# unilight/jatts

Hardware: AMD Instinct MI355X
Metric: audio samples/sec (22.05 kHz) + RTF, FastSpeech2+HiFi-GAN (higher is better)
Workload: dtype f32 (emulated: 3 exact bf16 terms per operand, 7 MFMA products, f32 accumulate; attention / norms / duration predictor exact f32); 1 GPU; FastSpeech2(JSUT conformer 4+4, adim 384)+HiFi-GAN v1 22k, 64 utts x 128 phonemes x 6 frames per GPU; hop=256, parallelism=dp1 (utterance sharding, int16 PCM all-gather)

## Files before the change

include/jatts_hip.h:

```cpp
#ifndef JATTS_HIP_H_
#define JATTS_HIP_H_

#include <stdint.h>

#ifdef __cplusplus
extern "C" {
#endif

#define JATTS_ABI_VERSION 4

#define JATTS_F32 0
#define JATTS_F16 1
#define JATTS_F32S 2
#define JATTS_F32E 3
#define JATTS_F32E6 4

#define JATTS_ACT_NONE 0
#define JATTS_ACT_RELU 1
#define JATTS_ACT_TANH 2
#define JATTS_ACT_SWISH 3
#define JATTS_ACT_MISH 4
#define JATTS_ACT_SNAKEBETA 5

#define JATTS_PAD_ZERO 0
#define JATTS_PAD_REFLECT 1

#define JATTS_PRE_NONE 0
#define JATTS_PRE_LRELU 1

#define JATTS_OK 0
#define JATTS_ERR_ARG (-1)
#define JATTS_ERR_HIP (-2)
#define JATTS_ERR_UNSUPPORTED (-3)

int jatts_abi_version(void);
const char* jatts_last_error(void);
int jatts_device_info(char* buf, int buflen);

typedef struct jatts_ragged {
  const int32_t* cu_rows;
  int32_t n_seq;
  int32_t max_len;
  int32_t len_mul;
  int32_t total_rows;
  const int32_t* host_lens;
} jatts_ragged;

typedef struct jatts_conv_desc {
  jatts_ragged rg;
  int32_t dtype;
  int32_t n_in;
  const void* x[3];
  int32_t ldx;
  float in_scale;
  int32_t pre_act;
  float pre_slope;
  const void* w;
  int32_t c_in;
  int32_t n_out;
  int32_t k_w;
  int32_t dil;
  int32_t pad;
  const float* bias;
  int32_t act;
  float alpha;
  const float* resid;
  int32_t ldr;
  void* y;
  int32_t ldy;
  int32_t y_is_f32;
  int32_t y_transposed;
  const int32_t* y_seq_col0;
  int32_t pad_mode;
  int32_t variant;
  const float* w_inv;
  const float* act_a;
  const float* act_b;
  int32_t n_split;
  int32_t ldy2;
  void* y2;
  const int32_t* y2_seq_col0;
  int32_t w_layout;
} jatts_conv_desc;

int jatts_conv1d(const jatts_conv_desc* d, void* stream);

int64_t jatts_conv_weight_index(int32_t n, int32_t tap, int32_t c, int32_t n_pad, int32_t c_in);

typedef struct jatts_resunit_desc {
  jatts_ragged rg;
  int32_t dtype;
  int32_t channels;
  int32_t k_w;
  int32_t dil;
  float slope;
  const void* x;
  void* y;
  const void* w1;
  const float* b1;
  const void* w2;
  const float* b2;
  const void* add0;
  const void* add1;
  float out_scale;
  const float* ws1;
  const float* ws2;
  int32_t w_layout;
} jatts_resunit_desc;

int jatts_hifigan_resunit(const jatts_resunit_desc* d, void* stream);

int64_t jatts_unit_weight_index_k32(int32_t n, int32_t tap, int32_t c, int32_t channels);

typedef struct jatts_resblock_desc {
  jatts_ragged rg;
  int32_t dtype;
  int32_t channels;
  int32_t k_w;
  int32_t n_units;
  int32_t dil[3];
  float slope;
  const void* x;
  void* y;
  const void* w1[3];
  const float* b1[3];
  const void* w2[3];
  const float* b2[3];
  const void* add0;
  const void* add1;
  float out_scale;
  const float* ws1[3];
  const float* ws2[3];
} jatts_resblock_desc;

int jatts_hifigan_resblock(const jatts_resblock_desc* d, void* stream);

int jatts_masked_loss(const jatts_ragged* rg, const float* a, int32_t lda, const float* b, int32_t ldb, int32_t dim,
                      const int32_t* valid_len, int32_t kind, float log_offset, double scale, float* out, double* workspace,
                      void* stream);
int jatts_conv1d_wgrad(const jatts_ragged* rg, const float* x, int32_t ldx, const float* dy, int32_t ldy, int32_t c_in,
                       int32_t n_out, int32_t k_w, int32_t dil, int32_t pad, float* dw, float* db, float* workspace, void* stream);
int jatts_pack_conv_weight(const float* w, int32_t n_out, int32_t c_in, int32_t k_w, int32_t c_mult, int32_t mode, int32_t dtype,
                           void* out, void* stream);
int jatts_pack_conv_weight_split(const float* w, int32_t n_out, int32_t c_in, int32_t k_w, int32_t c_mult, int32_t mode, void* out, float* inv,
                                 void* stream);
int jatts_col_sum(const float* x, int32_t ld, int64_t rows, int32_t dim, float* out, void* stream);

int jatts_layernorm_bwd(const float* x, int32_t ldx, const float* dy, int32_t lddy, const float* gamma, int64_t rows, int32_t dim,
                        float eps, float* dx, int32_t lddx, float* dgamma, float* dbeta, void* stream);
int jatts_act_fwd(int32_t mode, const float* x, float* y, int64_t n, void* stream);
int jatts_act_bwd(int32_t mode, const float* x, const float* dy, float* dx, int64_t n, void* stream);
int jatts_glu_fwd(const float* x, float* y, int64_t rows, int32_t dim, void* stream);
int jatts_glu_bwd(const float* x, const float* dy, float* dx, int64_t rows, int32_t dim, void* stream);
int jatts_dwconv(const jatts_ragged* rg, const float* x, const float* w, const float* bias, float* y, int32_t dim, int32_t k_w,
                 int32_t pad, int32_t flip, void* stream);
int jatts_dwconv_wgrad(const jatts_ragged* rg, const float* x, const float* dy, float* dw, int32_t dim, int32_t k_w, int32_t pad,
                       void* stream);
int jatts_col_stats(const float* x, const float* y2, int32_t ld, int64_t rows, int32_t dim, const float* shift, const float* mul,
                    int32_t mode, float* out0, float* out1, void* stream);
int jatts_bn_bwd_apply(const float* x, const float* dy, int64_t rows, int32_t dim, const float* mean, const float* rstd,
                       const float* gamma, const float* s_dy, const float* s_dyx, float* dx, void* stream);
int jatts_index_add_rows(const float* src, int32_t ld, const int64_t* idx, int64_t rows, int32_t dim, float scale, int64_t skip,
                         int64_t n_dst, float* dst, void* stream);
int jatts_lr_segment_sum(const jatts_ragged* rg, const int64_t* cum, const int32_t* cu_out, const float* dy, int32_t dim, float* dhs,
                         void* stream);
int jatts_shift_softmax_fwd(const float* ac, const float* bd, int32_t n_batch, int32_t n_heads, int32_t t_len, const int32_t* lens,
                            float scale, int32_t shift_mode, float* p, void* stream);
int jatts_shift_softmax_bwd(const float* p, const float* dp, int32_t n_batch, int32_t n_heads, int32_t t_len, float scale,
                            int32_t shift_mode, float* ds, float* dbd, void* stream);
int jatts_gate_bwd(const float* x, const float* dy, float* dx, int64_t rows, int32_t dim, void* stream);
int jatts_weight_norm_fwd(const float* v, const float* g, int32_t n_out, int32_t row_len, float* w, float* inv_norm, void* stream);
int jatts_weight_norm_bwd(const float* v, const float* g, const float* inv_norm, const float* dw, int32_t n_out, int32_t row_len,
                          float* dv, float* dg, void* stream);
int jatts_split_add(const float* o, const float* h, const float* skip, int64_t rows, int32_t dim, float* h_out, float* skip_out, void* stream);
int jatts_concat2(const float* a, const float* b, int64_t rows, int32_t dim, float* out, void* stream);
int jatts_outer_rows(const float* v, const float* w, const float* bias, int64_t rows, int32_t dim, int32_t accumulate, float* out,
                     void* stream);
int jatts_col_wsum(const float* x, int32_t ld, const float* v, int64_t rows, int32_t dim, float* out, void* stream);
int jatts_row_dot(const float* x, int32_t ld, const float* w, const float* bias, int64_t rows, int32_t dim, float* y, void* stream);
int jatts_masked_loss_bwd(const jatts_ragged* rg, const float* a, int32_t lda, const float* b, int32_t ldb, int32_t dim,
                          const int32_t* valid_len, int32_t kind, float log_offset, float scale, const float* upstream, float* da,
                          int32_t ldda, void* stream);
int jatts_groupnorm_fwd(const jatts_ragged* rg, const float* x, int32_t dim, int32_t groups, const float* gamma, const float* beta,
                        float eps, float* y, float* mean, float* rstd, void* stream);
int jatts_groupnorm_bwd(const jatts_ragged* rg, const float* x, const float* dy, int32_t dim, int32_t groups, const float* gamma,
                        const float* mean, const float* rstd, float* dx, float* dgamma, float* dbeta, void* stream);
int jatts_snakebeta_fwd(const float* x, float* y, int64_t rows, int32_t dim, const float* alpha, const float* beta, void* stream);
int jatts_snakebeta_bwd(const float* x, const float* dy, int64_t rows, int32_t dim, const float* alpha, const float* beta, float* dx,
                        float* dalpha, float* dbeta, void* stream);
int jatts_ctc_forward_sum(const float* log_p, int32_t n_batch, int32_t t_max, int32_t ld, const int32_t* ilens, const int32_t* olens,
                          int32_t max_ilen, float log_blank, float* workspace, float* nll, float* grad, float grad_scale, void* stream);
int jatts_seq_sum(const jatts_ragged* rg, const float* x, int32_t dim, float* out, void* stream);
int jatts_dropout(const float* x, float* y, int64_t n, float p, uint64_t seed, const uint64_t* seed_dev, void* stream);
int jatts_qkv_split(const float* qkv, const float* u, const float* v, int32_t n_batch, int32_t t_len, int32_t n_heads, int32_t d_k, float* qu,
                    float* qv, float* k, float* vv, void* stream);
int jatts_qkv_split_bwd(const float* dqu, const float* dqv, const float* dk, const float* dvv, int32_t n_batch, int32_t t_len, int32_t n_heads,
                        int32_t d_k, float* dqkv, float* du, float* dv, void* stream);
int jatts_act_dropout(int32_t mode, const float* x, const float* dy, float* out, int64_t n, float p, uint64_t seed, const uint64_t* seed_dev,
                      void* stream);
int jatts_dropout_add(const float* x, const float* resid, float* y, int64_t n, float p, float alpha, uint64_t seed, const uint64_t* seed_dev,
                      void* stream);
int jatts_gather_grads(const float* const* src, const int64_t* numel, const int64_t* dst_off, int32_t n, float* flat, int32_t accumulate,
                       void* stream);
int jatts_sumsq(const float* x, int64_t n, double* out, void* stream);
int jatts_adam_step(float* p, const float* g, float* m, float* v, int64_t n, double lr, double beta1, double beta2, double eps,
                    double weight_decay, int64_t step, const double* grad_sumsq, float max_norm, const float* hyper_dev, void* stream);

int jatts_debug_trace(void* buf, int64_t n_workgroups);

int jatts_mfma_probe(int32_t dtype, int32_t feed, const void* operands, int64_t operand_bytes, int32_t iters, int32_t workgroups,
                     uint64_t* clocks, float* sink, void* stream);
double jatts_mfma_probe_flops(int32_t dtype, int32_t iters, int32_t workgroups);

int jatts_bgemm(const float* a, int64_t sa_outer, int64_t sa_inner, int32_t lda, int32_t trans_a, const float* b, int64_t sb_outer,
                int64_t sb_inner, int32_t ldb, int32_t trans_b, float* c, int64_t sc_outer, int64_t sc_inner, int32_t ldc, int32_t n_outer,
                int32_t n_inner, int32_t m, int32_t n, int32_t k, float alpha, int32_t accumulate, void* stream);

int jatts_set_workspace(void* buf, int64_t bytes);

int jatts_hifigan_output(const jatts_ragged* rg, int32_t dtype, const void* const* x, int32_t n_in,
                         float in_scale, float slope, int32_t c_in, int32_t k_w, const float* w,
                         float bias, float* y, void* stream);

typedef struct jatts_relattn_desc {
  jatts_ragged rg;
  int32_t dtype;
  int32_t n_heads;
  int32_t d_k;
  const void* q;  int32_t ldq;
  const void* k;  int32_t ldk;
  const void* vt; int32_t ldvt;
  const void* g;  int32_t ldg;
  const float* ku;
  float scale;
  void* out; int32_t ldo;
  int32_t rel_mode;
  int32_t rel_center;
  const int32_t* vt_col0;
  const int32_t* kv_len;
} jatts_relattn_desc;

int jatts_relpos_attention(const jatts_relattn_desc* d, void* stream);

int jatts_rowdot(int32_t dtype, const void* x, int32_t ldx, int64_t rows, int32_t n_heads,
                 int32_t d_k, const float* vec, float* out, void* stream);

int jatts_embed_scale(const int64_t* ids, int64_t rows, const float* table, int32_t dim,
                      float scale, float* out, int64_t vocab, int64_t* n_bad, void* stream);

int jatts_layernorm(const void* x, int32_t in_dtype, int32_t ldx, void* y, int32_t out_dtype,
                    int32_t ldy, int64_t rows, int32_t dim, const float* gamma,
                    const float* beta, float eps, void* stream);

int jatts_affine_cast(const float* x, int32_t ldx, void* y, int32_t out_dtype, int32_t ldy,
                      int64_t rows, int32_t dim, const float* scale, const float* shift,
                      void* stream);
int jatts_affine_slice(const float* x, int32_t ldx, void* y, int32_t out_dtype, int32_t ldy,
                      int64_t rows, int32_t dim, const float* scale, const float* shift,
                      void* stream);

int jatts_glu_dwconv_bn_swish(const jatts_ragged* rg, int32_t dtype, const void* x, void* y,
                              int32_t channels, int32_t k_w, const float* w_dw,
                              const float* bn_scale, const float* bn_shift, void* stream);

int jatts_predictor_head(int32_t dtype, const void* x, int32_t ldx, int64_t rows, int32_t dim,
                         const float* w, float b, float* v_out, int64_t* dur_out, float offset,
                         void* stream);

int jatts_variance_embed_add(const jatts_ragged* rg, float* hs, int32_t dim, const float* p,
                             const float* wp, const float* bp, int32_t kp, const float* e,
                             const float* we, const float* be, int32_t ke, void* stream);

int jatts_gated_tanh_sigmoid(const jatts_ragged* rg, int32_t dtype, const void* x, const float* gseq,
                             void* y, int32_t channels, void* stream);

int jatts_groupnorm_mish(const jatts_ragged* rg, const void* x, int32_t in_dtype, void* y, int32_t out_dtype,
                         int32_t channels, int32_t groups, const float* gamma, const float* beta, float eps,
                         const float* addvec, float* workspace, void* stream);

int jatts_snakebeta(int32_t dtype, const void* x, void* y, int64_t rows, int32_t channels, const float* alpha,
                    const float* inv_beta, void* stream);

int jatts_l2_normalize(const float* x, int32_t ldx, void* y, int32_t out_dtype, int32_t ldy, int64_t rows,
                       int32_t dim, float eps, void* stream);

int jatts_gaussian_sample(const float* stats, const float* noise, float* z, int64_t rows, int32_t channels,
                          float noise_scale, void* stream);

int jatts_flip_channels(const float* x, float* y, int64_t rows, int32_t channels, void* stream);

int jatts_add_seq_vector(const jatts_ragged* rg, float* hs, int32_t dim, const float* vec,
                         void* stream);

int jatts_frame_signal(const jatts_ragged* rg_frames, const int32_t* cu_samples, const float* x, const float* window,
                       int32_t n_fft, int32_t hop, float* out, int32_t ldo, void* stream);
int jatts_power_spectrum(const float* x, int32_t ldx, int32_t n_bins, int64_t rows, float* out, int32_t ldo, void* stream);
int jatts_fbank_post(const jatts_ragged* rg, const float* p, int32_t ldp, int32_t n_mels, float amin, float top_db,
                     float* out, int32_t ldo, void* stream);
int jatts_seq_mean_std(const jatts_ragged* rg, const float* x, int32_t ldx, int32_t dim, const float* logits, int32_t ldl,
                       float* mean, float* stdv, int32_t ldm, float eps, void* stream);
int jatts_seq_affine_act(const jatts_ragged* rg, const float* x, int32_t ldx, int32_t dim, const float* seq_vec, int32_t pre_act,
                         const float* scale, const float* shift, int32_t post_act, void* y, int32_t out_dtype, int32_t ldy,
                         void* stream);
int jatts_se_scale_add(const jatts_ragged* rg, const float* x, int32_t dim, const float* s, const float* resid, float* y, int32_t ldy,
                       void* stream);

int jatts_lr_durations(const jatts_ragged* rg, const int64_t* d, float alpha, int32_t zero_rule,
                       int64_t* d_eff, int64_t* cum, int64_t* olens, void* stream);
int jatts_lr_gather(const jatts_ragged* rg_in, const int64_t* cum, const int32_t* cu_out,
                    int32_t max_out_len, const float* x, int32_t dim, float* out,
                    int64_t* frame_index, void* stream);

int jatts_zero_pad_rows(const jatts_ragged* rg, void* x, int32_t dtype, int32_t ld, int32_t dim, const int32_t* valid_len,
                        void* stream);
int jatts_cfm_mix(const jatts_ragged* rg, const float* x1, const float* z, const float* t, float sigma_min, int32_t dim,
                  float* y, float* u, void* stream);
int jatts_sq_err_sum(const float* a, const float* b, int64_t n, float scale, float* out, double* workspace, void* stream);

int jatts_gaussian_upsample(const jatts_ragged* rg_in, const int64_t* d, const int32_t* cu_out,
                            int32_t max_out_len, const float* hs, int32_t dim, float delta,
                            float* out, void* stream);

int jatts_pcm16(const float* x, int64_t n, int16_t* y, void* stream);

int jatts_alignment_logp(const jatts_ragged* rg_feats, const int32_t* cu_text, int32_t max_text_len, const float* feats,
                         const float* text, int32_t adim, float* log_p, int32_t ld, void* stream);

int jatts_mas_viterbi(const jatts_ragged* rg_feats, const int32_t* cu_text, const float* log_p, int32_t ld,
                      int32_t max_text_len, int64_t* path, int64_t* dur, double* score, void* stream);

#ifdef __cplusplus
}
#endif
#endif
```

jatts_amd/_abi.py:

```python
import ctypes as C
import os

_HERE = os.path.dirname(os.path.abspath(__file__))
LIB_PATH = os.environ.get("JATTS_HIP_LIB") or os.path.join(_HERE, "lib", "libjatts_hip.so")

F32, F16, F32S, F32E, F32E6 = 0, 1, 2, 3, 4
ABI_VERSION = 4
ACT_NONE, ACT_RELU, ACT_TANH, ACT_SWISH, ACT_MISH, ACT_SNAKEBETA = 0, 1, 2, 3, 4, 5
PRE_NONE, PRE_LRELU = 0, 1
PAD_ZERO, PAD_REFLECT = 0, 1


class Ragged(C.Structure):
    _fields_ = [("cu_rows", C.c_void_p), ("n_seq", C.c_int32), ("max_len", C.c_int32),
                ("len_mul", C.c_int32), ("total_rows", C.c_int32), ("host_lens", C.c_void_p)]


class ConvDesc(C.Structure):
    _fields_ = [
        ("rg", Ragged), ("dtype", C.c_int32), ("n_in", C.c_int32), ("x", C.c_void_p * 3),
        ("ldx", C.c_int32), ("in_scale", C.c_float), ("pre_act", C.c_int32), ("pre_slope", C.c_float),
        ("w", C.c_void_p), ("c_in", C.c_int32), ("n_out", C.c_int32), ("k_w", C.c_int32),
        ("dil", C.c_int32), ("pad", C.c_int32), ("bias", C.c_void_p), ("act", C.c_int32),
        ("alpha", C.c_float), ("resid", C.c_void_p), ("ldr", C.c_int32), ("y", C.c_void_p),
        ("ldy", C.c_int32), ("y_is_f32", C.c_int32), ("y_transposed", C.c_int32), ("y_seq_col0", C.c_void_p),
        ("pad_mode", C.c_int32), ("variant", C.c_int32), ("w_inv", C.c_void_p), ("act_a", C.c_void_p), ("act_b", C.c_void_p),
        ("n_split", C.c_int32), ("ldy2", C.c_int32), ("y2", C.c_void_p), ("y2_seq_col0", C.c_void_p), ("w_layout", C.c_int32),
    ]


class ResUnitDesc(C.Structure):
    _fields_ = [
        ("rg", Ragged), ("dtype", C.c_int32), ("channels", C.c_int32), ("k_w", C.c_int32),
        ("dil", C.c_int32), ("slope", C.c_float), ("x", C.c_void_p), ("y", C.c_void_p),
        ("w1", C.c_void_p), ("b1", C.c_void_p), ("w2", C.c_void_p), ("b2", C.c_void_p),
        ("add0", C.c_void_p), ("add1", C.c_void_p), ("out_scale", C.c_float),
        ("ws1", C.c_void_p), ("ws2", C.c_void_p), ("w_layout", C.c_int32),
    ]


class ResBlockDesc(C.Structure):
    _fields_ = [
        ("rg", Ragged), ("dtype", C.c_int32), ("channels", C.c_int32), ("k_w", C.c_int32), ("n_units", C.c_int32),
        ("dil", C.c_int32 * 3), ("slope", C.c_float), ("x", C.c_void_p), ("y", C.c_void_p),
        ("w1", C.c_void_p * 3), ("b1", C.c_void_p * 3), ("w2", C.c_void_p * 3), ("b2", C.c_void_p * 3),
        ("add0", C.c_void_p), ("add1", C.c_void_p), ("out_scale", C.c_float),
        ("ws1", C.c_void_p * 3), ("ws2", C.c_void_p * 3),
    ]


class RelAttnDesc(C.Structure):
    _fields_ = [
        ("rg", Ragged), ("dtype", C.c_int32), ("n_heads", C.c_int32), ("d_k", C.c_int32),
        ("q", C.c_void_p), ("ldq", C.c_int32), ("k", C.c_void_p), ("ldk", C.c_int32),
        ("vt", C.c_void_p), ("ldvt", C.c_int32), ("g", C.c_void_p), ("ldg", C.c_int32),
        ("ku", C.c_void_p), ("scale", C.c_float), ("out", C.c_void_p), ("ldo", C.c_int32),
        ("rel_mode", C.c_int32), ("rel_center", C.c_int32), ("vt_col0", C.c_void_p), ("kv_len", C.c_void_p),
    ]


PROTOTYPES = {
    "jatts_abi_version": (C.c_int, []),
    "jatts_last_error": (C.c_char_p, []),
    "jatts_device_info": (C.c_int, [C.c_char_p, C.c_int]),
    "jatts_conv1d": (C.c_int, [C.POINTER(ConvDesc), C.c_void_p]),
    "jatts_conv_weight_index": (C.c_int64, [C.c_int32] * 5),
    "jatts_hifigan_resunit": (C.c_int, [C.POINTER(ResUnitDesc), C.c_void_p]),
    "jatts_unit_weight_index_k32": (C.c_int64, [C.c_int32] * 4),
    "jatts_hifigan_resblock": (C.c_int, [C.POINTER(ResBlockDesc), C.c_void_p]),
    "jatts_debug_trace": (C.c_int, [C.c_void_p, C.c_int64]),
    "jatts_mfma_probe": (C.c_int, [C.c_int32, C.c_int32, C.c_void_p, C.c_int64, C.c_int32, C.c_int32, C.c_void_p, C.c_void_p, C.c_void_p]),
    "jatts_mfma_probe_flops": (C.c_double, [C.c_int32, C.c_int32, C.c_int32]),
    "jatts_set_workspace": (C.c_int, [C.c_void_p, C.c_int64]),
    "jatts_pack_conv_weight_split": (C.c_int, [C.c_void_p, C.c_int32, C.c_int32, C.c_int32, C.c_int32, C.c_int32, C.c_void_p, C.c_void_p, C.c_void_p]),
    "jatts_bgemm": (C.c_int, [C.c_void_p, C.c_int64, C.c_int64, C.c_int32, C.c_int32, C.c_void_p, C.c_int64, C.c_int64, C.c_int32, C.c_int32,
                              C.c_void_p, C.c_int64, C.c_int64, C.c_int32, C.c_int32, C.c_int32, C.c_int32, C.c_int32, C.c_int32, C.c_float,
                              C.c_int32, C.c_void_p]),
    "jatts_pcm16": (C.c_int, [C.c_void_p, C.c_int64, C.c_void_p, C.c_void_p]),
    "jatts_alignment_logp": (C.c_int, [C.POINTER(Ragged), C.c_void_p, C.c_int32, C.c_void_p, C.c_void_p, C.c_int32,
                                       C.c_void_p, C.c_int32, C.c_void_p]),
    "jatts_mas_viterbi": (C.c_int, [C.POINTER(Ragged), C.c_void_p, C.c_void_p, C.c_int32, C.c_int32, C.c_void_p,
                                    C.c_void_p, C.c_void_p, C.c_void_p]),
    "jatts_hifigan_output": (C.c_int, [C.POINTER(Ragged), C.c_int32, C.POINTER(C.c_void_p), C.c_int32,
                                       C.c_float, C.c_float, C.c_int32, C.c_int32, C.c_void_p, C.c_float,
                                       C.c_void_p, C.c_void_p]),
    "jatts_relpos_attention": (C.c_int, [C.POINTER(RelAttnDesc), C.c_void_p]),
    "jatts_rowdot": (C.c_int, [C.c_int32, C.c_void_p, C.c_int32, C.c_int64, C.c_int32, C.c_int32,
                               C.c_void_p, C.c_void_p, C.c_void_p]),
    "jatts_embed_scale": (C.c_int, [C.c_void_p, C.c_int64, C.c_void_p, C.c_int32, C.c_float, C.c_void_p,
                                    C.c_int64, C.c_void_p, C.c_void_p]),
    "jatts_layernorm": (C.c_int, [C.c_void_p, C.c_int32, C.c_int32, C.c_void_p, C.c_int32, C.c_int32,
                                  C.c_int64, C.c_int32, C.c_void_p, C.c_void_p, C.c_float, C.c_void_p]),
    "jatts_affine_cast": (C.c_int, [C.c_void_p, C.c_int32, C.c_void_p, C.c_int32, C.c_int32, C.c_int64,
                                    C.c_int32, C.c_void_p, C.c_void_p, C.c_void_p]),
    "jatts_affine_slice": (C.c_int, [C.c_void_p, C.c_int32, C.c_void_p, C.c_int32, C.c_int32, C.c_int64,
                                     C.c_int32, C.c_void_p, C.c_void_p, C.c_void_p]),
    "jatts_glu_dwconv_bn_swish": (C.c_int, [C.POINTER(Ragged), C.c_int32, C.c_void_p, C.c_void_p, C.c_int32,
                                            C.c_int32, C.c_void_p, C.c_void_p, C.c_void_p, C.c_void_p]),
    "jatts_predictor_head": (C.c_int, [C.c_int32, C.c_void_p, C.c_int32, C.c_int64, C.c_int32, C.c_void_p,
                                       C.c_float, C.c_void_p, C.c_void_p, C.c_float, C.c_void_p]),
    "jatts_variance_embed_add": (C.c_int, [C.POINTER(Ragged), C.c_void_p, C.c_int32, C.c_void_p, C.c_void_p,
                                           C.c_void_p, C.c_int32, C.c_void_p, C.c_void_p, C.c_void_p,
                                           C.c_int32, C.c_void_p]),
    "jatts_gated_tanh_sigmoid": (C.c_int, [C.POINTER(Ragged), C.c_int32, C.c_void_p, C.c_void_p, C.c_void_p,
                                           C.c_int32, C.c_void_p]),
    "jatts_groupnorm_mish": (C.c_int, [C.POINTER(Ragged), C.c_void_p, C.c_int32, C.c_void_p, C.c_int32, C.c_int32,
                                       C.c_int32, C.c_void_p, C.c_void_p, C.c_float, C.c_void_p, C.c_void_p, C.c_void_p]),
    "jatts_snakebeta": (C.c_int, [C.c_int32, C.c_void_p, C.c_void_p, C.c_int64, C.c_int32, C.c_void_p, C.c_void_p,
                                  C.c_void_p]),
    "jatts_l2_normalize": (C.c_int, [C.c_void_p, C.c_int32, C.c_void_p, C.c_int32, C.c_int32, C.c_int64, C.c_int32,
                                     C.c_float, C.c_void_p]),
    "jatts_gaussian_sample": (C.c_int, [C.c_void_p, C.c_void_p, C.c_void_p, C.c_int64, C.c_int32, C.c_float,
                                        C.c_void_p]),
    "jatts_flip_channels": (C.c_int, [C.c_void_p, C.c_void_p, C.c_int64, C.c_int32, C.c_void_p]),
    "jatts_add_seq_vector": (C.c_int, [C.POINTER(Ragged), C.c_void_p, C.c_int32, C.c_void_p, C.c_void_p]),
    "jatts_lr_durations": (C.c_int, [C.POINTER(Ragged), C.c_void_p, C.c_float, C.c_int32, C.c_void_p,
                                     C.c_void_p, C.c_void_p, C.c_void_p]),
    "jatts_lr_gather": (C.c_int, [C.POINTER(Ragged), C.c_void_p, C.c_void_p, C.c_int32, C.c_void_p,
                                  C.c_int32, C.c_void_p, C.c_void_p, C.c_void_p]),
    "jatts_frame_signal": (C.c_int, [C.POINTER(Ragged), C.c_void_p, C.c_void_p, C.c_void_p, C.c_int32, C.c_int32, C.c_void_p,
                                     C.c_int32, C.c_void_p]),
    "jatts_power_spectrum": (C.c_int, [C.c_void_p, C.c_int32, C.c_int32, C.c_int64, C.c_void_p, C.c_int32, C.c_void_p]),
    "jatts_fbank_post": (C.c_int, [C.POINTER(Ragged), C.c_void_p, C.c_int32, C.c_int32, C.c_float, C.c_float, C.c_void_p,
                                   C.c_int32, C.c_void_p]),
    "jatts_seq_mean_std": (C.c_int, [C.POINTER(Ragged), C.c_void_p, C.c_int32, C.c_int32, C.c_void_p, C.c_int32, C.c_void_p,
                                     C.c_void_p, C.c_int32, C.c_float, C.c_void_p]),
    "jatts_seq_affine_act": (C.c_int, [C.POINTER(Ragged), C.c_void_p, C.c_int32, C.c_int32, C.c_void_p, C.c_int32, C.c_void_p,
                                       C.c_void_p, C.c_int32, C.c_void_p, C.c_int32, C.c_int32, C.c_void_p]),
    "jatts_se_scale_add": (C.c_int, [C.POINTER(Ragged), C.c_void_p, C.c_int32, C.c_void_p, C.c_void_p, C.c_void_p, C.c_int32,
                                     C.c_void_p]),
    "jatts_masked_loss": (C.c_int, [C.POINTER(Ragged), C.c_void_p, C.c_int32, C.c_void_p, C.c_int32, C.c_int32, C.c_void_p,
                                    C.c_int32, C.c_float, C.c_double, C.c_void_p, C.c_void_p, C.c_void_p]),
    "jatts_conv1d_wgrad": (C.c_int, [C.POINTER(Ragged), C.c_void_p, C.c_int32, C.c_void_p, C.c_int32, C.c_int32, C.c_int32,
                                     C.c_int32, C.c_int32, C.c_int32, C.c_void_p, C.c_void_p, C.c_void_p, C.c_void_p]),
    "jatts_pack_conv_weight": (C.c_int, [C.c_void_p, C.c_int32, C.c_int32, C.c_int32, C.c_int32, C.c_int32, C.c_int32, C.c_void_p, C.c_void_p]),
    "jatts_col_sum": (C.c_int, [C.c_void_p, C.c_int32, C.c_int64, C.c_int32, C.c_void_p, C.c_void_p]),
    "jatts_layernorm_bwd": (C.c_int, [C.c_void_p, C.c_int32, C.c_void_p, C.c_int32, C.c_void_p, C.c_int64, C.c_int32, C.c_float, C.c_void_p, C.c_int32, C.c_void_p, C.c_void_p, C.c_void_p]),
    "jatts_act_fwd": (C.c_int, [C.c_int32, C.c_void_p, C.c_void_p, C.c_int64, C.c_void_p]),
    "jatts_act_bwd": (C.c_int, [C.c_int32, C.c_void_p, C.c_void_p, C.c_void_p, C.c_int64, C.c_void_p]),
    "jatts_glu_fwd": (C.c_int, [C.c_void_p, C.c_void_p, C.c_int64, C.c_int32, C.c_void_p]),
    "jatts_glu_bwd": (C.c_int, [C.c_void_p, C.c_void_p, C.c_void_p, C.c_int64, C.c_int32, C.c_void_p]),
    "jatts_dwconv": (C.c_int, [C.POINTER(Ragged), C.c_void_p, C.c_void_p, C.c_void_p, C.c_void_p, C.c_int32, C.c_int32, C.c_int32, C.c_int32, C.c_void_p]),
    "jatts_dwconv_wgrad": (C.c_int, [C.POINTER(Ragged), C.c_void_p, C.c_void_p, C.c_void_p, C.c_int32, C.c_int32, C.c_int32, C.c_void_p]),
    "jatts_col_stats": (C.c_int, [C.c_void_p, C.c_void_p, C.c_int32, C.c_int64, C.c_int32, C.c_void_p, C.c_void_p, C.c_int32, C.c_void_p, C.c_void_p, C.c_void_p]),
    "jatts_bn_bwd_apply": (C.c_int, [C.c_void_p, C.c_void_p, C.c_int64, C.c_int32, C.c_void_p, C.c_void_p, C.c_void_p, C.c_void_p, C.c_void_p, C.c_void_p, C.c_void_p]),
    "jatts_index_add_rows": (C.c_int, [C.c_void_p, C.c_int32, C.c_void_p, C.c_int64, C.c_int32, C.c_float, C.c_int64, C.c_int64, C.c_void_p, C.c_void_p]),
    "jatts_lr_segment_sum": (C.c_int, [C.POINTER(Ragged), C.c_void_p, C.c_void_p, C.c_void_p, C.c_int32, C.c_void_p, C.c_void_p]),
    "jatts_shift_softmax_fwd": (C.c_int, [C.c_void_p, C.c_void_p, C.c_int32, C.c_int32, C.c_int32, C.c_void_p, C.c_float, C.c_int32, C.c_void_p, C.c_void_p]),
    "jatts_shift_softmax_bwd": (C.c_int, [C.c_void_p, C.c_void_p, C.c_int32, C.c_int32, C.c_int32, C.c_float, C.c_int32, C.c_void_p, C.c_void_p, C.c_void_p]),
    "jatts_gate_bwd": (C.c_int, [C.c_void_p, C.c_void_p, C.c_void_p, C.c_int64, C.c_int32, C.c_void_p]),
    "jatts_weight_norm_fwd": (C.c_int, [C.c_void_p, C.c_void_p, C.c_int32, C.c_int32, C.c_void_p, C.c_void_p, C.c_void_p]),
    "jatts_weight_norm_bwd": (C.c_int, [C.c_void_p, C.c_void_p, C.c_void_p, C.c_void_p, C.c_int32, C.c_int32, C.c_void_p, C.c_void_p, C.c_void_p]),
    "jatts_split_add": (C.c_int, [C.c_void_p, C.c_void_p, C.c_void_p, C.c_int64, C.c_int32, C.c_void_p, C.c_void_p, C.c_void_p]),
    "jatts_concat2": (C.c_int, [C.c_void_p, C.c_void_p, C.c_int64, C.c_int32, C.c_void_p, C.c_void_p]),
    "jatts_outer_rows": (C.c_int, [C.c_void_p, C.c_void_p, C.c_void_p, C.c_int64, C.c_int32, C.c_int32, C.c_void_p, C.c_void_p]),
    "jatts_col_wsum": (C.c_int, [C.c_void_p, C.c_int32, C.c_void_p, C.c_int64, C.c_int32, C.c_void_p, C.c_void_p]),
    "jatts_row_dot": (C.c_int, [C.c_void_p, C.c_int32, C.c_void_p, C.c_void_p, C.c_int64, C.c_int32, C.c_void_p, C.c_void_p]),
    "jatts_masked_loss_bwd": (C.c_int, [C.POINTER(Ragged), C.c_void_p, C.c_int32, C.c_void_p, C.c_int32, C.c_int32, C.c_void_p, C.c_int32, C.c_float, C.c_float, C.c_void_p, C.c_void_p, C.c_int32, C.c_void_p]),
    "jatts_groupnorm_fwd": (C.c_int, [C.POINTER(Ragged), C.c_void_p, C.c_int32, C.c_int32, C.c_void_p, C.c_void_p, C.c_float, C.c_void_p, C.c_void_p, C.c_void_p, C.c_void_p]),
    "jatts_groupnorm_bwd": (C.c_int, [C.POINTER(Ragged), C.c_void_p, C.c_void_p, C.c_int32, C.c_int32, C.c_void_p, C.c_void_p, C.c_void_p, C.c_void_p, C.c_void_p, C.c_void_p, C.c_void_p]),
    "jatts_snakebeta_fwd": (C.c_int, [C.c_void_p, C.c_void_p, C.c_int64, C.c_int32, C.c_void_p, C.c_void_p, C.c_void_p]),
    "jatts_snakebeta_bwd": (C.c_int, [C.c_void_p, C.c_void_p, C.c_int64, C.c_int32, C.c_void_p, C.c_void_p, C.c_void_p, C.c_void_p, C.c_void_p, C.c_void_p]),
    "jatts_ctc_forward_sum": (C.c_int, [C.c_void_p, C.c_int32, C.c_int32, C.c_int32, C.c_void_p, C.c_void_p, C.c_int32, C.c_float, C.c_void_p, C.c_void_p, C.c_void_p, C.c_float, C.c_void_p]),
    "jatts_seq_sum": (C.c_int, [C.POINTER(Ragged), C.c_void_p, C.c_int32, C.c_void_p, C.c_void_p]),
    "jatts_dropout": (C.c_int, [C.c_void_p, C.c_void_p, C.c_int64, C.c_float, C.c_uint64, C.c_void_p, C.c_void_p]),
    "jatts_qkv_split": (C.c_int, [C.c_void_p, C.c_void_p, C.c_void_p, C.c_int32, C.c_int32, C.c_int32, C.c_int32, C.c_void_p, C.c_void_p, C.c_void_p, C.c_void_p, C.c_void_p]),
    "jatts_qkv_split_bwd": (C.c_int, [C.c_void_p, C.c_void_p, C.c_void_p, C.c_void_p, C.c_int32, C.c_int32, C.c_int32, C.c_int32, C.c_void_p, C.c_void_p, C.c_void_p, C.c_void_p]),
    "jatts_act_dropout": (C.c_int, [C.c_int32, C.c_void_p, C.c_void_p, C.c_void_p, C.c_int64, C.c_float, C.c_uint64, C.c_void_p, C.c_void_p]),
    "jatts_dropout_add": (C.c_int, [C.c_void_p, C.c_void_p, C.c_void_p, C.c_int64, C.c_float, C.c_float, C.c_uint64, C.c_void_p, C.c_void_p]),
    "jatts_sumsq": (C.c_int, [C.c_void_p, C.c_int64, C.c_void_p, C.c_void_p]),
    "jatts_gather_grads": (C.c_int, [C.c_void_p, C.c_void_p, C.c_void_p, C.c_int32, C.c_void_p, C.c_int32, C.c_void_p]),
    "jatts_adam_step": (C.c_int, [C.c_void_p, C.c_void_p, C.c_void_p, C.c_void_p, C.c_int64, C.c_double, C.c_double, C.c_double, C.c_double, C.c_double, C.c_int64, C.c_void_p, C.c_float, C.c_void_p, C.c_void_p]),
    "jatts_zero_pad_rows": (C.c_int, [C.POINTER(Ragged), C.c_void_p, C.c_int32, C.c_int32, C.c_int32, C.c_void_p, C.c_void_p]),
    "jatts_cfm_mix": (C.c_int, [C.POINTER(Ragged), C.c_void_p, C.c_void_p, C.c_void_p, C.c_float, C.c_int32, C.c_void_p,
                                C.c_void_p, C.c_void_p]),
    "jatts_sq_err_sum": (C.c_int, [C.c_void_p, C.c_void_p, C.c_int64, C.c_float, C.c_void_p, C.c_void_p, C.c_void_p]),
    "jatts_gaussian_upsample": (C.c_int, [C.POINTER(Ragged), C.c_void_p, C.c_void_p, C.c_int32, C.c_void_p,
                                          C.c_int32, C.c_float, C.c_void_p, C.c_void_p]),
}

_lib = None


class JattsHipError(RuntimeError):
    pass


def load():
    global _lib
    if _lib is not None:
        return _lib
    if not os.path.exists(LIB_PATH):
        raise JattsHipError(
            f"{LIB_PATH} not found: build it with `python -c 'import __graft_entry__ as g; g.build()'` "
            "or `make -C jatts_amd/csrc`.  jatts_amd has no CPU fallback."
        )
    lib = C.CDLL(LIB_PATH)
    for name, (res, args) in PROTOTYPES.items():
        fn = getattr(lib, name)
        fn.restype, fn.argtypes = res, args
    if lib.jatts_abi_version() != ABI_VERSION:
        raise JattsHipError(f"libjatts_hip.so ABI version {lib.jatts_abi_version()} != {ABI_VERSION} (include/jatts_hip.h): rebuild with __graft_entry__.build()")
    _lib = lib
    return lib


def check(rc, what=""):
    if rc != 0:
        msg = load().jatts_last_error().decode(errors="replace")
        raise JattsHipError(f"{what} failed (rc={rc}): {msg}")
```

jatts_amd/csrc/conv_api.hip:

```cpp
#include <stdlib.h>

#include "common.h"

unsigned long long* jatts_g_trace = nullptr;
unsigned jatts_g_trace_cap = 0;

int jatts_conv1d_f16(const jatts_conv_desc& d, hipStream_t s);
int jatts_conv1d_f32(const jatts_conv_desc& d, hipStream_t s);
int jatts_conv1d_split(const jatts_conv_desc& d, hipStream_t s);
int jatts_conv1d_emul(const jatts_conv_desc& d, hipStream_t s);
int jatts_resunit_f16_narrow(const jatts_resunit_desc& d, hipStream_t s);
int jatts_resunit_f16_wide(const jatts_resunit_desc& d, hipStream_t s);
int jatts_resunit_f32(const jatts_resunit_desc& d, hipStream_t s);
int jatts_resunit_split(const jatts_resunit_desc& d, hipStream_t s);
int jatts_resunit_emul(const jatts_resunit_desc& d, hipStream_t s);
int jatts_resblock_f16(const jatts_resblock_desc& d, hipStream_t s);
int jatts_resblock_f32(const jatts_resblock_desc& d, hipStream_t s);
int jatts_resblock_split(const jatts_resblock_desc& d, hipStream_t s);
int jatts_resblock_emul(const jatts_resblock_desc& d, hipStream_t s);

extern "C" int jatts_debug_trace(void* buf, int64_t n_workgroups) {
  jatts_g_trace = (unsigned long long*)buf;
  jatts_g_trace_cap = buf ? (unsigned)n_workgroups : 0u;
  return JATTS_OK;
}

extern "C" int64_t jatts_conv_weight_index(int32_t n, int32_t tap, int32_t c, int32_t n_pad, int32_t c_in) {
  const int64_t KC16 = c_in / 16, NFR = n_pad / 32;
  const int64_t kc = c / 16, nf = n / 32;
  const int64_t lane = 32 * ((c % 16) / 8) + (n % 32);
  return ((((int64_t)tap * KC16 + kc) * NFR + nf) * 64 + lane) * 8 + (c % 8);
}

extern "C" int64_t jatts_unit_weight_index_k32(int32_t n, int32_t tap, int32_t c, int32_t channels) {
  const int64_t KC32 = channels / 32, NFR16 = channels / 16;
  const int64_t kc = c / 32, nf = n / 16;
  const int64_t lane = 16 * ((c % 32) / 8) + (n % 16);
  return ((((int64_t)tap * KC32 + kc) * NFR16 + nf) * 64 + lane) * 8 + (c % 8);
}

extern "C" int jatts_conv1d(const jatts_conv_desc* d, void* stream) {
  if (!d || !d->x[0] || !d->w || !d->y || !d->rg.cu_rows) return jatts_set_error_msg(JATTS_ERR_ARG, "conv1d: null pointer");
  if (d->c_in <= 0 || d->c_in % 64) return jatts_set_error_msg(JATTS_ERR_ARG, "conv1d: c_in must be a positive multiple of 64");
  if (d->ldx % 8) return jatts_set_error_msg(JATTS_ERR_ARG, "conv1d: ldx must be a multiple of 8");
  if (d->n_in < 1 || d->n_in > 3 || d->k_w < 1 || d->dil < 1 || d->n_out < 1 || d->rg.n_seq < 1 || d->rg.len_mul < 1)
    return jatts_set_error_msg(JATTS_ERR_ARG, "conv1d: bad geometry");
  if (d->act == JATTS_ACT_SNAKEBETA && (!d->act_a || !d->act_b || (d->n_out & 3) || ((uintptr_t)d->act_a & 15) || ((uintptr_t)d->act_b & 15)))
    return jatts_set_error_msg(JATTS_ERR_ARG, "conv1d: JATTS_ACT_SNAKEBETA needs 16-byte aligned act_a / act_b and n_out % 4 == 0");
  if (d->n_split != 0 && (d->n_split < 0 || d->n_split % 256 || d->n_split >= d->n_out || !d->y2 || d->y_transposed || d->resid || d->ldy2 <= 0))
    return jatts_set_error_msg(JATTS_ERR_ARG, "conv1d: n_split must be a multiple of 256 below n_out, with y2 / ldy2 set, y row-major and no residual");
  if (d->w_layout != 0 && d->dtype != JATTS_F32E && d->dtype != JATTS_F32E6) return jatts_set_error_msg(JATTS_ERR_ARG, "conv1d: w_layout = 1 goes with JATTS_F32E / JATTS_F32E6 only");
  if (d->rg.max_len <= 0) return JATTS_OK;
  hipStream_t s = (hipStream_t)stream;
  if (d->dtype == JATTS_F16) return jatts_conv1d_f16(*d, s);
  if (d->dtype == JATTS_F32) return jatts_conv1d_f32(*d, s);
  if (d->dtype == JATTS_F32S) {
    if (!d->w_inv) return jatts_set_error_msg(JATTS_ERR_ARG, "conv1d: JATTS_F32S needs w_inv");
    if (!d->y_is_f32) return jatts_set_error_msg(JATTS_ERR_ARG, "conv1d: JATTS_F32S writes f32 (y_is_f32 = 1)");
    return jatts_conv1d_split(*d, s);
  }
  if (d->dtype == JATTS_F32E || d->dtype == JATTS_F32E6) {
    if (!d->y_is_f32) return jatts_set_error_msg(JATTS_ERR_ARG, "conv1d: JATTS_F32E / JATTS_F32E6 write f32 (y_is_f32 = 1)");
    if (d->w_layout != 0 && d->w_layout != 1) return jatts_set_error_msg(JATTS_ERR_ARG, "conv1d: w_layout must be 0 or 1");
    return jatts_conv1d_emul(*d, s);
  }
  return jatts_set_error_msg(JATTS_ERR_ARG, "conv1d: unknown dtype");
}

extern "C" int jatts_hifigan_resunit(const jatts_resunit_desc* d, void* stream) {
  if (!d || !d->x || !d->y || !d->w1 || !d->w2 || !d->b1 || !d->b2 || !d->rg.cu_rows)
    return jatts_set_error_msg(JATTS_ERR_ARG, "resunit: null pointer");
  if (d->x == d->y) return jatts_set_error_msg(JATTS_ERR_ARG, "resunit: y must not alias x");
  if (d->k_w < 1 || !(d->k_w & 1) || d->dil < 1) return jatts_set_error_msg(JATTS_ERR_ARG, "resunit: odd k_w and dil>=1 required");
  if (!(d->slope >= 0.f && d->slope <= 1.f)) return jatts_set_error_msg(JATTS_ERR_ARG, "resunit: LeakyReLU slope must be in [0, 1]");
  if (d->rg.max_len <= 0) return JATTS_OK;
  hipStream_t s = (hipStream_t)stream;
  if (d->dtype == JATTS_F16) return d->channels <= 64 ? jatts_resunit_f16_narrow(*d, s) : jatts_resunit_f16_wide(*d, s);
  if (d->dtype == JATTS_F32) return jatts_resunit_f32(*d, s);
  if (d->dtype == JATTS_F32S) {
    if (!d->ws1 || !d->ws2) return jatts_set_error_msg(JATTS_ERR_ARG, "resunit: JATTS_F32S needs ws1 / ws2");
    return jatts_resunit_split(*d, s);
  }
  if (d->dtype == JATTS_F32E || d->dtype == JATTS_F32E6) {
    if (d->w_layout != 0 && d->w_layout != 1) return jatts_set_error_msg(JATTS_ERR_ARG, "resunit: w_layout must be 0 or 1");
    return jatts_resunit_emul(*d, s);
  }
  if (d->w_layout != 0) return jatts_set_error_msg(JATTS_ERR_ARG, "resunit: w_layout = 1 goes with JATTS_F32E / JATTS_F32E6 only");
  return jatts_set_error_msg(JATTS_ERR_UNSUPPORTED, "resunit: unsupported channels/dtype (use jatts_conv1d)");
}

extern "C" int jatts_hifigan_resblock(const jatts_resblock_desc* d, void* stream) {
  if (!d || !d->x || !d->y || !d->rg.cu_rows) return jatts_set_error_msg(JATTS_ERR_ARG, "resblock: null pointer");
  if (d->n_units < 1 || d->n_units > 3) return jatts_set_error_msg(JATTS_ERR_ARG, "resblock: 1..3 units");
  for (int u = 0; u < d->n_units; ++u) {
    if (!d->w1[u] || !d->w2[u] || !d->b1[u] || !d->b2[u]) return jatts_set_error_msg(JATTS_ERR_ARG, "resblock: null weights");
    if (d->dil[u] < 1) return jatts_set_error_msg(JATTS_ERR_ARG, "resblock: dil >= 1 required");
  }
  if (d->x == d->y) return jatts_set_error_msg(JATTS_ERR_ARG, "resblock: y must not alias x");
  if (d->k_w < 1 || !(d->k_w & 1)) return jatts_set_error_msg(JATTS_ERR_ARG, "resblock: odd k_w required");
  if (!(d->slope >= 0.f && d->slope <= 1.f)) return jatts_set_error_msg(JATTS_ERR_ARG, "resblock: LeakyReLU slope must be in [0, 1]");
  if (d->dtype == JATTS_F32S) {
    for (int u = 0; u < d->n_units; ++u)
      if (!d->ws1[u] || !d->ws2[u]) return jatts_set_error_msg(JATTS_ERR_ARG, "resblock: JATTS_F32S needs ws1 / ws2");
    if (d->rg.max_len <= 0) return JATTS_OK;
    return jatts_resblock_split(*d, (hipStream_t)stream);
  }
  if (d->dtype == JATTS_F32E || d->dtype == JATTS_F32E6) {
    if (d->rg.max_len <= 0) return JATTS_OK;
    return jatts_resblock_emul(*d, (hipStream_t)stream);
  }
  if (d->dtype != JATTS_F16 && d->dtype != JATTS_F32) return jatts_set_error_msg(JATTS_ERR_ARG, "resblock: unknown dtype");
  if (d->rg.max_len <= 0) return JATTS_OK;
  return d->dtype == JATTS_F16 ? jatts_resblock_f16(*d, (hipStream_t)stream) : jatts_resblock_f32(*d, (hipStream_t)stream);
}
```

jatts_amd/csrc/resunit_emul.hip:

```cpp
#include "resunit_emul16_impl.h"

template <typename T>
static int resunit_emul(const jatts_resunit_desc& d, hipStream_t s) {
  const int halo = (d.k_w - 1) * d.dil;
  const int64_t cols = (int64_t)d.rg.max_len * d.rg.len_mul;
  auto wgs = [&](int window) { const int64_t tt = window - (d.k_w - 1); return tt > 0 ? ((cols + tt - 1) / tt) * d.rg.n_seq : (int64_t)1 << 40; };
  switch (d.channels) {
    case 32: return launch_resunit_emul<T, 32, 256, 1, 2, 2, 2, false, true>(d, s);
    case 64:
      if (d.k_w >= 11) return launch_resunit_emul<T, 64, 256, 1, 2, 2, 1, false, true>(d, s);
      return launch_resunit_emul<T, 64, 128, 2, 2, 2, 2, false, true>(d, s);
    case 128:
      if (wgs(128) <= 448 && (64 + halo) * 784 + 1024 <= 80 * 1024) return launch_resunit_emul<T, 128, 64, 2, 1, 2, 2>(d, s);
      return launch_resunit_emul<T, 128, 128, 2, 2, 2, 1>(d, s);
    case 256:
      if (wgs(64) <= 160) return launch_resunit_emul<T, 256, 32, 4, 1, 2, 1>(d, s);
      if ((64 + halo) * 1552 + 2048 <= 160 * 1024) return launch_resunit_emul<T, 256, 64, 4, 2, 2, 1>(d, s);
      return launch_resunit_emul<T, 256, 64, 4, 2, 2, 1, true>(d, s);
  }
  return jatts_set_error_msg(JATTS_ERR_UNSUPPORTED, "resunit: unsupported channels for JATTS_F32E (32 / 64 / 128 / 256)");
}

template <typename T>
static int resunit_emul16(const jatts_resunit_desc& d, hipStream_t s) {
  const int halo = (d.k_w - 1) * d.dil;
  switch (d.channels) {
    case 32: return launch_resunit_emul16<T, 32, 256, 1, 4, 2, false, true>(d, s);
    case 64:
      if (d.k_w >= 11) return launch_resunit_emul16<T, 64, 256, 1, 4, 1, false, true>(d, s);
      return launch_resunit_emul16<T, 64, 128, 2, 2, 2, false, true>(d, s);
    case 128: return launch_resunit_emul16<T, 128, 128, 2, 2, 1>(d, s);
    case 256:
      if ((64 + halo) * 1552 + 2048 <= 160 * 1024) return launch_resunit_emul16<T, 256, 64, 4, 1, 1>(d, s);
      return launch_resunit_emul16<T, 256, 64, 4, 1, 1, true>(d, s);
  }
  return jatts_set_error_msg(JATTS_ERR_UNSUPPORTED, "resunit: unsupported channels for JATTS_F32E (32 / 64 / 128 / 256)");
}

int jatts_resunit_emul(const jatts_resunit_desc& d, hipStream_t s) {
  if (d.w_layout == 1) return d.dtype == JATTS_F32E6 ? resunit_emul16<bf3f>(d, s) : resunit_emul16<bf3>(d, s);
  return d.dtype == JATTS_F32E6 ? resunit_emul<bf3f>(d, s) : resunit_emul<bf3>(d, s);
}
```

jatts_amd/csrc/resunit_emul16_impl.h:

```cpp
#pragma once
#include <type_traits>

#include "resunit_emul_impl.h"

#ifndef JATTS_U16_ROWS
#define JATTS_U16_ROWS 1
#endif
#ifndef JATTS_U16_DIAG
#define JATTS_U16_DIAG 0
#endif

namespace {

struct acc2x4 { f32x4 big, small; };
template <typename T> struct Acc16 { typedef f32x4 type; };
template <> struct Acc16<bf3p<7>> { typedef acc2x4 type; };
__device__ __forceinline__ void acc16_set(f32x4& a, int i, float v) { a[i] = v; }
__device__ __forceinline__ void acc16_set(acc2x4& a, int i, float v) { a.small[i] = v; a.big[i] = 0.f; }
__device__ __forceinline__ void acc16_finish(f32x4&) {}
__device__ __forceinline__ void acc16_finish(acc2x4& a) { a.small = a.big + a.small; }
__device__ __forceinline__ f32x4& acc16_val(f32x4& a) { return a; }
__device__ __forceinline__ f32x4& acc16_val(acc2x4& a) { return a.small; }

template <int P> __device__ __forceinline__ void mma16p(const bf3px8<7>& a, const bf3px8<7>& b, acc2x4& c) {
  if constexpr (P == 0) c.small = __builtin_amdgcn_mfma_f32_16x16x32_bf16(a.b1, b.b2, c.small, 0, 0, 0);
  if constexpr (P == 1) c.small = __builtin_amdgcn_mfma_f32_16x16x32_bf16(a.b2, b.b0, c.small, 0, 0, 0);
  if constexpr (P == 2) c.small = __builtin_amdgcn_mfma_f32_16x16x32_bf16(a.b0, b.b2, c.small, 0, 0, 0);
  if constexpr (P == 3) c.small = __builtin_amdgcn_mfma_f32_16x16x32_bf16(a.b1, b.b1, c.small, 0, 0, 0);
  if constexpr (P == 4) c.small = __builtin_amdgcn_mfma_f32_16x16x32_bf16(a.b1, b.b0, c.small, 0, 0, 0);
  if constexpr (P == 5) c.small = __builtin_amdgcn_mfma_f32_16x16x32_bf16(a.b0, b.b1, c.small, 0, 0, 0);
  if constexpr (P == 6) c.big = __builtin_amdgcn_mfma_f32_16x16x32_bf16(a.b0, b.b0, c.big, 0, 0, 0);
}
template <int P> __device__ __forceinline__ void mma16p(const bf3px8<6>& a, const bf3px8<6>& b, f32x4& c) {
  if constexpr (P == 0) c = __builtin_amdgcn_mfma_f32_16x16x32_bf16(a.b2, b.b0, c, 0, 0, 0);
  if constexpr (P == 1) c = __builtin_amdgcn_mfma_f32_16x16x32_bf16(a.b0, b.b2, c, 0, 0, 0);
  if constexpr (P == 2) c = __builtin_amdgcn_mfma_f32_16x16x32_bf16(a.b1, b.b1, c, 0, 0, 0);
  if constexpr (P == 3) c = __builtin_amdgcn_mfma_f32_16x16x32_bf16(a.b1, b.b0, c, 0, 0, 0);
  if constexpr (P == 4) c = __builtin_amdgcn_mfma_f32_16x16x32_bf16(a.b0, b.b1, c, 0, 0, 0);
  if constexpr (P == 5) c = __builtin_amdgcn_mfma_f32_16x16x32_bf16(a.b0, b.b0, c, 0, 0, 0);
}
template <typename T> struct NProd;
template <int NP> struct NProd<bf3p<NP>> { static constexpr int value = NP; };

template <typename T, int NF>
struct WStream16 {
  typedef typename Elem<T>::vec8 V8;
  V8 ra[NF];
  const T* wl;
  int kc_stride;
  int tap_stride;
  __device__ __forceinline__ void bind(const T* w, int KC32, int NFR16, int nf0, int lane) {
    wl = w + (size_t)nf0 * 512 + (size_t)lane * 8;
    kc_stride = NFR16 * 512;
    tap_stride = KC32 * kc_stride;
  }
  __device__ __forceinline__ void fetch(int tap, int kc) {
    const T* p = wl + (size_t)tap * tap_stride + (size_t)kc * kc_stride;
#pragma unroll
    for (int f = 0; f < NF; ++f) ra[f] = Vec8IO<T>::ldg(p + f * 512);
  }
};

template <typename T, int NF, int NT>
__device__ __forceinline__ void pair16(typename Acc16<T>::type (&acc)[NF][NT], const typename Elem<T>::vec8& a, typename Elem<T>::vec8 (&rb)[NT], int f_, int t0_) {
  constexpr int NP = NProd<T>::value;
  auto& c0 = acc[f_][t0_];
  auto& c1 = acc[f_][t0_ + 1];
  mma16p<0>(a, rb[t0_], c0); mma16p<0>(a, rb[t0_ + 1], c1);
  mma16p<1>(a, rb[t0_], c0); mma16p<1>(a, rb[t0_ + 1], c1);
  mma16p<2>(a, rb[t0_], c0); mma16p<2>(a, rb[t0_ + 1], c1);
  mma16p<3>(a, rb[t0_], c0); mma16p<3>(a, rb[t0_ + 1], c1);
  mma16p<4>(a, rb[t0_], c0); mma16p<4>(a, rb[t0_ + 1], c1);
  mma16p<5>(a, rb[t0_], c0); mma16p<5>(a, rb[t0_ + 1], c1);
  if constexpr (NP == 7) { mma16p<6>(a, rb[t0_], c0); mma16p<6>(a, rb[t0_ + 1], c1); }
}

template <typename T, int NF, int NT>
__device__ __forceinline__ void row16(typename Acc16<T>::type (&acc)[NF][NT], const typename Elem<T>::vec8& a, typename Elem<T>::vec8 (&rb)[NT], int f_) {
  constexpr int NP = NProd<T>::value;
#pragma unroll
  for (int t = 0; t < NT; ++t) mma16p<0>(a, rb[t], acc[f_][t]);
#pragma unroll
  for (int t = 0; t < NT; ++t) mma16p<1>(a, rb[t], acc[f_][t]);
#pragma unroll
  for (int t = 0; t < NT; ++t) mma16p<2>(a, rb[t], acc[f_][t]);
#pragma unroll
  for (int t = 0; t < NT; ++t) mma16p<3>(a, rb[t], acc[f_][t]);
#pragma unroll
  for (int t = 0; t < NT; ++t) mma16p<4>(a, rb[t], acc[f_][t]);
#pragma unroll
  for (int t = 0; t < NT; ++t) mma16p<5>(a, rb[t], acc[f_][t]);
  if constexpr (NP == 7) {
#pragma unroll
    for (int t = 0; t < NT; ++t) mma16p<6>(a, rb[t], acc[f_][t]);
  }
}

template <typename T, int NF, int NT>
__device__ __forceinline__ void step16(typename Acc16<T>::type (&acc)[NF][NT], typename Elem<T>::vec8 (&ra)[NF], typename Elem<T>::vec8 (&rb)[NT], const T* pa,
                                       const char* pb, int pitch) {
  static_assert(NT % 2 == 0, "column fragments come in pairs");
  constexpr bool ROWS16 = JATTS_U16_ROWS != 0;
#pragma unroll
  for (int f = 0; f < NF; ++f) {
    if (f < NF - 1 && ROWS16) {
      row16<T, NF, NT>(acc, ra[f], rb, f);
      __builtin_amdgcn_sched_barrier(0);
    } else {
#pragma unroll
      for (int tp = 0; tp < NT; tp += 2) {
        pair16<T, NF, NT>(acc, ra[f], rb, f, tp);
        if (f == NF - 1 && !(JATTS_U16_DIAG & 1)) {
          rb[tp] = Vec8IO<T>::lds(pb + (size_t)(tp * 16) * pitch);
          rb[tp + 1] = Vec8IO<T>::lds(pb + (size_t)((tp + 1) * 16) * pitch);
        }
        __builtin_amdgcn_sched_barrier(0);
      }
    }
    if (!(JATTS_U16_DIAG & 2)) ra[f] = Vec8IO<T>::ldg(pa + f * 512);
    __builtin_amdgcn_sched_barrier(0);
  }
}

template <typename T, int NF, int NT, int KCS>
__device__ __forceinline__ void conv16(typename Acc16<T>::type (&acc)[NF][NT], WStream16<T, NF>& ws, int kc0, int k_w, int dil, const char* act, int pitch,
                                       int col0, int lane, const T* tail) {
  typedef typename Elem<T>::vec8 V8;
  const int steps = k_w * KCS;
  const char* bbase = act + (size_t)(col0 + (lane & 15)) * pitch + (size_t)(lane >> 4) * 48;
  const T* abase = ws.wl + (size_t)kc0 * ws.kc_stride;
  V8 rb[NT];
#pragma unroll
  for (int t = 0; t < NT; ++t) rb[t] = Vec8IO<T>::lds(bbase + (size_t)(t * 16) * pitch);
  __builtin_amdgcn_sched_barrier(0);
  if (!tail) tail = abase + (size_t)(k_w - 1) * ws.tap_stride + (size_t)(KCS - 1) * ws.kc_stride;
  int tap = 0, kk = 0;
  for (int s = 0; s < steps; ++s) {
    int nkk = kk + 1;
    const bool wrap = nkk == KCS;
    nkk = wrap ? 0 : nkk;
    const int ntap = tap + (wrap ? 1 : 0);
    const bool last = s + 1 >= steps;
    const T* pa = last ? tail : abase + (size_t)ntap * ws.tap_stride + (size_t)nkk * ws.kc_stride;
    const char* pb = bbase + (size_t)((last ? tap : ntap) * dil) * pitch + (size_t)((last ? kk : nkk) * 4) * 48;
    step16<T, NF, NT>(acc, ws.ra, rb, pa, pb, pitch);
    tap = ntap;
    kk = nkk;
  }
}

template <typename T, int C, int WGCOLS, int WN, int WT, int OCC, bool KSPLIT = false, bool RREG = false>
__global__ __launch_bounds__(WN* WT * 64, OCC) void resunit_emul16_kernel(jatts_resunit_desc d, unsigned long long* trace, unsigned trace_cap,
                                                                         unsigned bias_off) {
  typedef typename Elem<T>::vec8 V8;
  extern __shared__ __attribute__((aligned(16))) char smem[];
  constexpr int NF = C / (WN * 16), NT = WGCOLS / (WT * 16);
  constexpr int KC32 = C / 32, NFR16 = C / 16;
  constexpr int pitch = C * 6 + 16;
  constexpr int pitch_x = KSPLIT ? (C / 2) * 6 + 16 : pitch;
  constexpr int NTHR = WN * WT * 64;
  static_assert(NF * WN * 16 == C && NT * WT * 16 == WGCOLS && C % 32 == 0, "tile shape");
  static_assert(sizeof(T) == 6, "bf3 is three packed bf16");
  static_assert(!(KSPLIT && RREG), "the residual registers go with the one-piece x tile");
  static_assert(!KSPLIT || KC32 % 2 == 0, "channel halves are whole K-steps");
  constexpr int MAXI = RREG ? (WGCOLS * (C / 8) + NTHR - 1) / NTHR : 1;
  f32x8 xk[MAXI];
  const unsigned wg_lin = blockIdx.x + blockIdx.y * gridDim.x;
  const bool tracing = trace != nullptr && wg_lin < trace_cap && threadIdx.x == 0;
#define JATTS_STAMP(i) do { if (tracing) trace[(size_t)wg_lin * 16 + (i)] = __builtin_amdgcn_s_memtime(); } while (0)
  if (tracing) {
    unsigned hwid, xcc;
    asm volatile("s_getreg_b32 %0, hwreg(HW_REG_HW_ID)" : "=s"(hwid));
    asm volatile("s_getreg_b32 %0, hwreg(HW_REG_XCC_ID)" : "=s"(xcc));
    trace[(size_t)wg_lin * 16] = ((unsigned long long)xcc << 32) | hwid;
    trace[(size_t)wg_lin * 16 + 8] = __builtin_amdgcn_s_memrealtime();
  }
  JATTS_STAMP(1);
  const int K = d.k_w, dil = d.dil;
  const int p2 = (K - 1) / 2, p1 = p2 * dil;
  const int tt_out = WGCOLS - 2 * p2;

  int b = blockIdx.y, bx = blockIdx.x;
  if (ragged_is_1d(d.rg) && !ragged_locate(d.rg, tt_out, blockIdx.x, b, bx)) return;
  const int row_b = d.rg.cu_rows[b];
  const int L = (d.rg.cu_rows[b + 1] - row_b) * d.rg.len_mul;
  const int t0 = bx * tt_out;
  if (t0 >= L) return;
  const int64_t seq_row0 = (int64_t)row_b * d.rg.len_mul;
  const int lane = threadIdx.x & 63, wave = threadIdx.x >> 6;
  const int wn = wave / WT, wt = wave % WT;
  const int g4 = lane >> 4;
  const int col0 = wt * NT * 16;
  const int nf0 = wn * NF;

  const int rx = WGCOLS + 2 * p1;
  char* xs = smem;
  char* hs = smem;
  float* bs = reinterpret_cast<float*>(smem + bias_off);
  for (int u = threadIdx.x; u < 2 * C; u += NTHR) bs[u] = u < C ? d.b1[u] : d.b2[u - C];

  WStream16<T, NF> ws;
  ws.bind((const T*)d.w1, KC32, NFR16, nf0, lane);
  ws.fetch(0, 0);

  typename Acc16<T>::type acc[NF][NT];
  auto bias_acc = [&](const float* bv) {
#pragma unroll
    for (int f = 0; f < NF; ++f) {
      const f32x4 bb = *reinterpret_cast<const f32x4*>(bv + (nf0 + f) * 16 + 4 * g4);
#pragma unroll
      for (int t = 0; t < NT; ++t)
#pragma unroll
        for (int e = 0; e < 4; ++e) acc16_set(acc[f][t], e, bb[e]);
    }
  };
  auto finish_acc = [&]() {
#pragma unroll
    for (int f = 0; f < NF; ++f)
#pragma unroll
      for (int t = 0; t < NT; ++t) acc16_finish(acc[f][t]);
  };
  auto to_planes = [&](f32x8 v) {
    lrelu8(v, d.slope);
    V8 o;
    bf3_split8(v, o);
    return o;
  };
  const float* x = (const float*)d.x;
  const int pos0 = t0 - p2 - p1;
  if constexpr (!KSPLIT) {
    constexpr int UPR = C / 8;
    constexpr int UB = 8;
    const int total = rx * UPR;
    if constexpr (RREG) {
      const int r_in = p1 + p2, n_in = tt_out * UPR;
#pragma unroll
      for (int j = 0; j < MAXI; ++j) {
        const int v = threadIdx.x + j * NTHR;
        const int ro = v / UPR, cu = v - ro * UPR;
        const int pos = t0 + ro;
        if (v < n_in && pos < L) xk[j] = Vec8IO<float>::ldg(x + (seq_row0 + pos) * (int64_t)C + cu * 8);
        else xk[j] = f32x8{0, 0, 0, 0, 0, 0, 0, 0};
      }
      const int n_halo = (rx - tt_out) * UPR;
      for (int base = threadIdx.x; base < n_halo; base += NTHR * UB) {
        f32x8 v[UB];
#pragma unroll
        for (int j = 0; j < UB; ++j) {
          const int u = base + j * NTHR;
          int r = u / UPR;
          const int cu = u - r * UPR;
          if (r >= r_in) r += tt_out;
          const int pos = pos0 + r;
          if (u < n_halo && pos >= 0 && pos < L) v[j] = Vec8IO<float>::ldg(x + (seq_row0 + pos) * (int64_t)C + cu * 8);
          else v[j] = f32x8{0, 0, 0, 0, 0, 0, 0, 0};
        }
#pragma unroll
        for (int j = 0; j < UB; ++j) {
          const int u = base + j * NTHR;
          if (u >= n_halo) continue;
          int r = u / UPR;
          const int cu = u - r * UPR;
          if (r >= r_in) r += tt_out;
          Vec8IO<T>::sts(xs + (size_t)r * pitch + (size_t)cu * 48, to_planes(v[j]));
        }
      }
#pragma unroll
      for (int j = 0; j < MAXI; ++j) {
        const int v = threadIdx.x + j * NTHR;
        if (v >= n_in) continue;
        const int ro = v / UPR, cu = v - ro * UPR;
        Vec8IO<T>::sts(xs + (size_t)(r_in + ro) * pitch + (size_t)cu * 48, to_planes(xk[j]));
      }
    } else {
      constexpr int UBX = ((WGCOLS + 64) * UPR + NTHR - 1) / NTHR;
      for (int base = threadIdx.x; base < total; base += NTHR * UBX) {
        f32x8 v[UBX];
#pragma unroll
        for (int j = 0; j < UBX; ++j) {
          const int u = base + j * NTHR;
          const int r = u / UPR, cu = u - r * UPR;
          const int pos = pos0 + r;
          if (u < total && pos >= 0 && pos < L) v[j] = Vec8IO<float>::ldg(x + (seq_row0 + pos) * (int64_t)C + cu * 8);
          else v[j] = f32x8{0, 0, 0, 0, 0, 0, 0, 0};
        }
#pragma unroll
        for (int j = 0; j < UBX; ++j) {
          const int u = base + j * NTHR;
          if (u >= total) continue;
          const int r = u / UPR, cu = u - r * UPR;
          Vec8IO<T>::sts(xs + (size_t)r * pitch + (size_t)cu * 48, to_planes(v[j]));
        }
      }
    }
    __syncthreads();
    JATTS_STAMP(2);
    bias_acc(bs);
    conv16<T, NF, NT, KC32>(acc, ws, 0, K, dil, xs, pitch, col0, lane, (const T*)d.w2 + (size_t)nf0 * 512 + (size_t)lane * 8);
  } else {
    constexpr int UPR = C / 16;
    constexpr int MAXU = ((WGCOLS + 64) * UPR + NTHR - 1) / NTHR;
    const int total = rx * UPR;
    f32x8 xv[MAXU];
    auto load_half = [&](int half) {
#pragma unroll
      for (int j = 0; j < MAXU; ++j) {
        const int u = threadIdx.x + j * NTHR;
        const int r = u / UPR, cu = u - r * UPR;
        const int pos = pos0 + r;
        if (u < total && pos >= 0 && pos < L) xv[j] = Vec8IO<float>::ldg(x + (seq_row0 + pos) * (int64_t)C + half * (C / 2) + cu * 8);
        else xv[j] = f32x8{0, 0, 0, 0, 0, 0, 0, 0};
      }
    };
    auto store_half = [&]() {
#pragma unroll
      for (int j = 0; j < MAXU; ++j) {
        const int u = threadIdx.x + j * NTHR;
        if (u < total) Vec8IO<T>::sts(xs + (size_t)(u / UPR) * pitch_x + (size_t)(u % UPR) * 48, to_planes(xv[j]));
      }
    };
    load_half(0);
    store_half();
    load_half(1);
    __syncthreads();
    JATTS_STAMP(2);
    bias_acc(bs);
    conv16<T, NF, NT, KC32 / 2>(acc, ws, 0, K, dil, xs, pitch_x, col0, lane, ws.wl + (size_t)(KC32 / 2) * ws.kc_stride);
    lds_barrier();
    store_half();
    lds_barrier();
    conv16<T, NF, NT, KC32 / 2>(acc, ws, KC32 / 2, K, dil, xs, pitch_x, col0, lane, (const T*)d.w2 + (size_t)nf0 * 512 + (size_t)lane * 8);
  }
  finish_acc();
  JATTS_STAMP(3);

  lds_barrier();
  JATTS_STAMP(10);
  for (int u = threadIdx.x; u < (K - 1) * (C / 8); u += NTHR) {
    const int r = WGCOLS + u / (C / 8), cu = u % (C / 8);
    V8 z;
#pragma unroll
    for (int e = 0; e < 8; ++e) z.b0[e] = z.b1[e] = z.b2[e] = (bf16)0.f;
    Vec8IO<T>::sts(hs + (size_t)r * pitch + (size_t)cu * 48, z);
  }
#pragma unroll
  for (int t = 0; t < NT; ++t) {
    const int col = col0 + t * 16 + (lane & 15);
    const int pos = t0 - p2 + col;
    const float keep = (pos >= 0 && pos < L) ? 1.f : 0.f;
#pragma unroll
    for (int f = 0; f < NF; ++f) {
      const int n0 = (nf0 + f) * 16 + 4 * g4;
      float v[4];
#pragma unroll
      for (int e = 0; e < 4; ++e) {
        const float a = acc16_val(acc[f][t])[e] * keep;
        v[e] = fmaxf(a, a * d.slope);
      }
      bf16x4 q0, q1, q2;
      bf3_split4(v, q0, q1, q2);
      char* p = hs + (size_t)col * pitch + (size_t)(n0 >> 3) * 48 + (size_t)(n0 & 4) * 2;
      *reinterpret_cast<bf16x4*>(p) = q0;
      *reinterpret_cast<bf16x4*>(p + 16) = q1;
      *reinterpret_cast<bf16x4*>(p + 32) = q2;
    }
  }
  JATTS_STAMP(12);
  lds_barrier();
  JATTS_STAMP(4);

  bias_acc(bs + C);
  ws.bind((const T*)d.w2, KC32, NFR16, nf0, lane);
  conv16<T, NF, NT, KC32>(acc, ws, 0, K, 1, hs, pitch, col0, lane, nullptr);
  finish_acc();
  JATTS_STAMP(5);

  __syncthreads();
  char* ys = smem;
#pragma unroll
  for (int t = 0; t < NT; ++t) {
    const int col = col0 + t * 16 + (lane & 15);
    if (col >= tt_out || t0 + col >= L) continue;
#pragma unroll
    for (int f = 0; f < NF; ++f) {
      const int n0 = (nf0 + f) * 16 + 4 * g4;
      *reinterpret_cast<f32x4*>(ys + (size_t)col * pitch + (size_t)n0 * 4) = acc16_val(acc[f][t]);
    }
  }
  __syncthreads();
  JATTS_STAMP(6);
  {
    const int vrows = min(tt_out, L - t0);
    const int64_t g0 = (seq_row0 + t0) * (int64_t)C;
    constexpr bool keep_small = C <= 64;
    const float* xg = (const float*)d.x;
    float* yg = (float*)d.y;
    if constexpr (RREG) {
      constexpr int UPR = C / 8;
      const int n_out = vrows * UPR;
      const bool has_add1 = d.add0 != nullptr && d.add1 != nullptr;
      f32x8 a0[MAXI], a1[MAXI];
      if (d.add0) {
#pragma unroll
        for (int j = 0; j < MAXI; ++j) {
          const int v = threadIdx.x + j * NTHR;
          if (v < n_out) {
            a0[j] = Vec8IO<float>::ldg((const float*)d.add0 + g0 + (int64_t)v * 8);
            if (has_add1) a1[j] = Vec8IO<float>::ldg((const float*)d.add1 + g0 + (int64_t)v * 8);
          }
        }
      }
#pragma unroll
      for (int j = 0; j < MAXI; ++j) {
        const int v = threadIdx.x + j * NTHR;
        if (v >= n_out) continue;
        const int ro = v / UPR, cu = v - ro * UPR;
        f32x8 o = Vec8IO<float>::lds(ys + (size_t)ro * pitch + (size_t)cu * 32);
#pragma unroll
        for (int e = 0; e < 8; ++e) o[e] = o[e] + xk[j][e];
        if (d.add0) {
#pragma unroll
          for (int e = 0; e < 8; ++e) o[e] = (o[e] + a0[j][e] + (has_add1 ? a1[j][e] : 0.f)) * d.out_scale;
        }
        float* dst = yg + g0 + (int64_t)v * 8;
        *reinterpret_cast<f32x4*>(dst) = f32x4{o[0], o[1], o[2], o[3]};
        *reinterpret_cast<f32x4*>(dst + 4) = f32x4{o[4], o[5], o[6], o[7]};
      }
    } else {
      if (d.add0) unit_store_pass<float, C, keep_small ? 2 : 4, true, NTHR>(d.add0, d.add1, d.out_scale, ys, pitch, vrows, xg, yg, g0);
      else unit_store_pass<float, C, keep_small ? 4 : 8, false, NTHR>(d.add0, d.add1, d.out_scale, ys, pitch, vrows, xg, yg, g0);
    }
  }
  JATTS_STAMP(7);
  if (tracing) trace[(size_t)wg_lin * 16 + 9] = __builtin_amdgcn_s_memrealtime();
#undef JATTS_STAMP
}

template <typename T, int C, int WGCOLS, int WN, int WT, int OCC = 2, bool KSPLIT = false, bool RREG = false>
int launch_resunit_emul16(const jatts_resunit_desc& d, hipStream_t s) {
  const int K = d.k_w, p2 = (K - 1) / 2, p1 = p2 * d.dil;
  const int tt_out = WGCOLS - 2 * p2;
  if (tt_out < 8) return jatts_set_error_msg(JATTS_ERR_UNSUPPORTED, "resunit: kernel too wide for tile");
  const size_t pitch = C * 6 + 16, pitch_x = KSPLIT ? (C / 2) * 6 + 16 : pitch;
  const size_t rows_x = WGCOLS + 2 * p1, rows_h = WGCOLS + K - 1;
  if (KSPLIT && 2 * p1 > 64) return jatts_set_error_msg(JATTS_ERR_UNSUPPORTED, "resunit (emulated, channel halves): halo beyond 32 rows a side");
  size_t lds = rows_x * pitch_x > rows_h * pitch ? rows_x * pitch_x : rows_h * pitch;
  const unsigned bias_off = (unsigned)lds;
  lds += 2 * C * sizeof(float);
  if (lds > 160 * 1024) return jatts_set_error_msg(JATTS_ERR_UNSUPPORTED, "resunit: tile exceeds 160 KiB LDS");
  const int64_t maxL = (int64_t)d.rg.max_len * d.rg.len_mul;
  dim3 grid((unsigned)((maxL + tt_out - 1) / tt_out), (unsigned)d.rg.n_seq);
  if (const int64_t n1 = ragged_tiles_1d(d.rg, tt_out)) grid = dim3((unsigned)n1);
  auto kern = resunit_emul16_kernel<T, C, WGCOLS, WN, WT, OCC, KSPLIT, RREG>;
  JATTS_RAISE_LDS_LIMIT(kern);
  hipLaunchKernelGGL(kern, grid, dim3(WN * WT * 64), lds, s, d, jatts_g_trace, jatts_g_trace_cap, bias_off);
  JATTS_CHECK_LAUNCH();
  return JATTS_OK;
}

}
```

jatts_amd/hip.py:

```python
import collections
import contextlib
import ctypes as C

import torch

from . import _abi
from ._abi import ACT_MISH, ACT_NONE, ACT_RELU, ACT_SWISH, ACT_TANH, F16, F32, F32E, F32E6, F32S

_TORCH = {F32: torch.float32, F16: torch.float16, F32S: torch.float32, F32E: torch.float32, F32E6: torch.float32}
EMUL = (F32E, F32E6)


def torch_dtype(code):
    return _TORCH[code]


def code_of(t):
    if t.dtype == torch.float32:
        return F32
    if t.dtype == torch.float16:
        return F16
    raise TypeError(f"unsupported dtype {t.dtype}")


_PROF = None


def profile_begin():
    global _PROF
    _PROF = []


def profile_end():
    global _PROF
    recs, _PROF = _PROF or [], None
    torch.cuda.synchronize()
    return [(tag, meta, a.elapsed_time(b)) for tag, meta, a, b in recs]


_FLOPS = None


def flops_begin():
    global _FLOPS
    _FLOPS = 0.0


def flops_end():
    global _FLOPS
    v, _FLOPS = _FLOPS or 0.0, None
    return v


def _count(flops):
    global _FLOPS
    if _FLOPS is not None:
        _FLOPS += flops


class _ZeroPool:
    def __init__(self, device, floats=1 << 20):
        self.buf = torch.zeros(floats, dtype=torch.float32, device=device)
        self.off, self.high, self.misses = 0, 0, 0
        self.active = False
        self._retired = []

    def begin(self):
        self.high = max(self.high, self.off)
        if self.high:
            self.buf[:self.high].zero_()
        self.off = 0

    def end(self):
        self.high = max(self.high, self.off)
        if self.misses:
            self._retired.append(self.buf)
            self.buf = torch.zeros(max(2 * self.buf.numel(), 2 * (self.high + self.misses)), dtype=torch.float32, device=self.buf.device)
            self.misses = 0

    def take(self, numel):
        n = (numel + 15) & ~15
        if self.off + n > self.buf.numel():
            self.misses += n
            return None
        t = self.buf[self.off:self.off + numel]
        self.off += n
        return t


_ZPOOL = None


def zero_pool_begin(device):
    global _ZPOOL
    dev = torch.device(device)
    if dev.index is None:
        dev = torch.device(dev.type, torch.cuda.current_device())
    if _ZPOOL is None or _ZPOOL.buf.device != dev:
        _ZPOOL = _ZeroPool(dev)
    _ZPOOL.begin()
    _ZPOOL.active = True


def zero_pool_end():
    if _ZPOOL is not None:
        _ZPOOL.active = False
        if not torch.cuda.is_current_stream_capturing():
            _ZPOOL.end()


def _zeros(shape, device):
    shape = (shape,) if isinstance(shape, int) else tuple(shape)
    if _ZPOOL is not None and getattr(_ZPOOL, "active", False) and _ZPOOL.buf.device == device:
        n = 1
        for v in shape:
            n *= v
        t = _ZPOOL.take(n)
        if t is not None:
            return t.view(shape)
    return torch.zeros(shape, dtype=torch.float32, device=device)


class _Timed:
    def __init__(self, tag, meta):
        self.tag, self.meta = tag, meta

    def __enter__(self):
        if _PROF is not None:
            self.a = torch.cuda.Event(enable_timing=True)
            self.a.record()

    def __exit__(self, *exc):
        if _PROF is not None:
            b = torch.cuda.Event(enable_timing=True)
            b.record()
            _PROF.append((self.tag, self.meta, self.a, b))


def _stream():
    return C.c_void_p(torch.cuda.current_stream().cuda_stream)


_WS = {}
_WS_CURRENT = [None]
_WS_OWNER = {}
WS_BYTES = 64 * 1024 + 96 * 1024 * 1024


def _ws(device):
    key = str(device)
    if not torch.cuda.is_current_stream_capturing():
        cur = torch.cuda.current_stream(device)
        own = _WS_OWNER.get(key)
        if own is not None and own[0] != cur.cuda_stream and not own[1].query():
            cur.wait_event(own[1])
        ev = own[1] if (own is not None and own[0] == cur.cuda_stream) else torch.cuda.Event()
        _WS_OWNER[key] = (cur.cuda_stream, ev)
        _WS_PENDING[0] = (cur, ev)
    if _WS_CURRENT[0] == key:
        return
    buf = _WS.get(key)
    if buf is None:
        if torch.cuda.is_current_stream_capturing():
            raise _abi.JattsHipError("the reduction scratch must exist before a graph capture: run one eager step first")
        buf = _WS[key] = torch.zeros(WS_BYTES, dtype=torch.uint8, device=device)
        torch.cuda.current_stream(device).synchronize()
    _abi.check(_abi.load().jatts_set_workspace(buf.data_ptr(), buf.numel()), "jatts_set_workspace")
    _WS_CURRENT[0] = key


_WS_PENDING = [None]


def _ws_done():
    p, _WS_PENDING[0] = _WS_PENDING[0], None
    if p is not None:
        p[1].record(p[0])


def _ws_check(rc, name):
    try:
        _abi.check(rc, name)
    finally:
        _ws_done()


def _ptr(t, col0=0):
    if t is None:
        return None
    return t.data_ptr() + col0 * t.element_size()


def _dev(t):
    if not t.is_cuda:
        raise _abi.JattsHipError("jatts_amd kernels need device tensors (no CPU fallback)")
    return t


_KEEP = [None]


def keep_begin():
    _KEEP[0] = []
    return _KEEP[0]


def keep_end():
    _KEEP[0] = None


def keep(t):
    if _KEEP[0] is not None and t is not None:
        _KEEP[0].append(t)
    return t


def h2d(values, dtype, device):
    dev = torch.device(device)
    if dev.type != "cuda":
        return torch.tensor(values, dtype=dtype, device=dev)
    key = None
    if isinstance(values, (list, tuple)) and len(values) <= 65536 and all(isinstance(v, (int, float, bool)) for v in values[:1] + values[-1:]):
        key = (tuple(values), dtype, dev.index if dev.index is not None else torch.cuda.current_device())
        hit = _H2D_CACHE.get(key)
        if hit is not None:
            _H2D_CACHE.move_to_end(key)
            if hit[2] != torch.cuda.current_stream().cuda_stream and not torch.cuda.is_current_stream_capturing() and not hit[1].query():
                torch.cuda.current_stream().wait_event(hit[1])
            return keep(hit[0])
    if torch.cuda.is_current_stream_capturing():
        raise _abi.JattsHipError("h2d of new values while a graph is being captured: run the step once outside the capture first")
    t = torch.tensor(values, dtype=dtype).pin_memory().to(dev, non_blocking=True)
    if key is not None:
        ev = torch.cuda.Event()
        ev.record()
        _H2D_CACHE[key] = (t, ev, torch.cuda.current_stream().cuda_stream)
        _H2D_BYTES[0] += t.numel() * t.element_size()
        while _H2D_BYTES[0] > _H2D_CACHE_MAX_BYTES and len(_H2D_CACHE) > 1:
            _, old = _H2D_CACHE.popitem(last=False)
            _H2D_BYTES[0] -= old[0].numel() * old[0].element_size()
    return keep(t)


_H2D_CACHE = collections.OrderedDict()
_H2D_BYTES = [0]
_H2D_CACHE_MAX_BYTES = 8 << 20
_GEOM_CACHE = {}
_GEOM_CACHE_MAX = 512


class RaggedBatch:

    def __init__(self, lens, device):
        self.lens = [int(v) for v in lens]
        cu = [0]
        for v in self.lens:
            cu.append(cu[-1] + v)
        self.cu_host = cu
        self.total = cu[-1]
        self.n_seq = len(self.lens)
        self.max_len = max(self.lens) if self.lens else 0
        self.device = device
        dev = torch.device(device)
        if dev.type != "cuda":
            self.cu = torch.tensor(cu, dtype=torch.int32, device=dev)
            return
        key = (tuple(self.lens), dev.index if dev.index is not None else torch.cuda.current_device())
        hit = _GEOM_CACHE.get(key)
        if hit is None:
            t = h2d(cu, torch.int32, dev)
            ev = torch.cuda.Event()
            ev.record()
            if len(_GEOM_CACHE) >= _GEOM_CACHE_MAX:
                _GEOM_CACHE.pop(next(iter(_GEOM_CACHE)))
            _GEOM_CACHE[key] = hit = (t, ev, torch.cuda.current_stream().cuda_stream)
        elif hit[2] != torch.cuda.current_stream().cuda_stream and not torch.cuda.is_current_stream_capturing() and not hit[1].query():
            torch.cuda.current_stream().wait_event(hit[1])
        self.cu = keep(hit[0])

    def struct(self, len_mul=1):
        if _RAGGED_1D and self.n_seq > 1 and min(self.lens) != self.max_len:
            if not hasattr(self, "_lens_c"):
                self._lens_c = (C.c_int32 * self.n_seq)(*self.lens)
            return _abi.Ragged(self.cu.data_ptr(), self.n_seq, self.max_len, len_mul, self.total, C.addressof(self._lens_c))
        return _abi.Ragged(self.cu.data_ptr(), self.n_seq, self.max_len, len_mul, 0, None)

    def vt_layout(self):
        if not hasattr(self, "_vt"):
            col, c = [], 0
            for v in self.lens:
                col.append(c)
                c += round_up(v, 8)
            self._vt = (h2d(col or [0], torch.int32, self.device), c + 8)
        return self._vt


_RAGGED_1D = True


def round_up(v, m):
    return (v + m - 1) // m * m


def pack_conv_weight(w, dtype_code, c_mult=64):
    n, c, k = w.shape
    n_pad, c_pad = round_up(n, 32), round_up(c, c_mult)
    wp = torch.zeros(n_pad, c_pad, k, dtype=torch.float32, device=w.device)
    wp[:n, :c] = w.float()
    wp = wp.permute(2, 0, 1).reshape(k, n_pad // 32, 32, c_pad // 16, 2, 8)
    wp = wp.permute(0, 3, 1, 4, 2, 5).contiguous().reshape(-1)
    return wp.to(torch_dtype(dtype_code))


def pack_conv_weight_split(w, c_mult=32):
    n, c, k = w.shape
    w = w.detach().float()
    n_pad = round_up(n, 32)
    amax = w.abs().reshape(n, -1).amax(dim=1)
    e = torch.frexp(amax)[1]
    s = torch.where(amax > 0, 15 - e, torch.zeros_like(e)).clamp(-60, 60).to(torch.int32)
    scale = ((127 + s) << 23).view(torch.float32)
    ws = w * scale.view(-1, 1, 1)
    hi = ws.half()
    lo = (ws - hi.float()).half()
    ph = pack_conv_weight(hi.float(), F16, c_mult).view(-1, 8)
    pl = pack_conv_weight(lo.float(), F16, c_mult).view(-1, 8)
    inv = torch.ones(n_pad, dtype=torch.float32, device=w.device)
    inv[:n] = ((127 - s) << 23).view(torch.float32)
    return torch.stack([ph, pl], dim=1).reshape(-1).contiguous(), inv.contiguous()


def bf16x3_terms(w):
    w = w.detach().float()
    b0 = w.bfloat16()
    r1 = w - b0.float()
    b1 = r1.bfloat16()
    b2 = (r1 - b1.float()).bfloat16()
    return b0, b1, b2


def pack_conv_weight_bf16x3(w, c_mult=32):
    planes = [pack_conv_weight(t.float(), F32, c_mult).view(-1, 8).bfloat16() for t in bf16x3_terms(w)]
    return torch.stack(planes, dim=1).reshape(-1).contiguous()


def pack_unit_weight_bf16x3_k32(w):
    n_out, c_in, k = w.shape
    if n_out % 16 or c_in % 32:
        raise ValueError("pack_unit_weight_bf16x3_k32: channels must be a multiple of 32")
    planes = []
    for t in bf16x3_terms(w):
        v = t.permute(2, 1, 0).reshape(k, c_in // 32, 4, 8, n_out // 16, 16).permute(0, 1, 4, 2, 5, 3)
        planes.append(v.reshape(-1, 8))
    return torch.stack(planes, dim=1).reshape(-1).contiguous()


def pack_conv_weight_bf16x3_k32(w, c_mult=64):
    n, c, k = w.shape
    n_pad, c_pad = round_up(n, 32), round_up(c, c_mult)
    wp = torch.zeros(n_pad, c_pad, k, dtype=torch.float32, device=w.device)
    wp[:n, :c] = w.detach().float()
    return pack_unit_weight_bf16x3_k32(wp)


class SplitWeight:

    def __init__(self, w, c_mult=64):
        self.packed, self.inv = pack_conv_weight_split(w, c_mult)
        self._src, self._c_mult, self._f32 = w.detach(), c_mult, None

    def f32(self):
        if self._f32 is None:
            self._f32 = pack_conv_weight(self._src, F32, self._c_mult)
        return self._f32


class EmulWeight:

    def __init__(self, w, c_mult=64, code=F32E, layout=None):
        self.code = code
        self.layout = (1 if c_mult % 64 == 0 else 0) if layout is None else layout
        self.packed = pack_conv_weight_bf16x3_k32(w, c_mult) if self.layout else pack_conv_weight_bf16x3(w, c_mult)
        self._src, self._c_mult, self._f32 = w.detach(), c_mult, None

    def f32(self):
        if self._f32 is None:
            self._f32 = pack_conv_weight(self._src, F32, self._c_mult)
        return self._f32


_SPLIT_WEIGHTS = [0]
WEIGHT_MODE = {"fp16": 0, "fp32": 0, "fp32_split": 1, "fp32_bf16x3": 2, "fp32_bf16x3_6p": 3}
EMUL_CODE = {2: F32E, 3: F32E6}
PRECISIONS = tuple(WEIGHT_MODE)


@contextlib.contextmanager
def split_weights(on=True):
    mode = WEIGHT_MODE[on] if isinstance(on, str) else int(on)
    prev, _SPLIT_WEIGHTS[0] = _SPLIT_WEIGHTS[0], mode
    try:
        yield
    finally:
        _SPLIT_WEIGHTS[0] = prev


def f32_operand(w, c_mult=64):
    m = _SPLIT_WEIGHTS[0]
    return SplitWeight(w, c_mult) if m == 1 else EmulWeight(w, c_mult, EMUL_CODE[m]) if m in EMUL_CODE else pack_conv_weight(w, F32, c_mult)


def pack_conv_weight_dev(w, dtype_code, c_mult=64, dgrad=False):
    lib = _abi.load()
    w = _dev(w)
    if w.dtype != torch.float32 or not w.is_contiguous():
        w = w.float().contiguous()
    n, c, k = w.shape
    pn, pc = (c, n) if dgrad else (n, c)
    n_pad, c_pad = round_up(pn, 32), round_up(pc, c_mult)
    out = torch.empty(k * n_pad * c_pad, dtype=torch_dtype(dtype_code), device=w.device)
    _abi.check(lib.jatts_pack_conv_weight(w.data_ptr(), n, c, k, c_mult, int(dgrad), dtype_code, out.data_ptr(), _stream()),
               "jatts_pack_conv_weight")
    return out, c_pad


def pack_conv_weight_split_dev(w, c_mult=64, dgrad=False):
    lib = _abi.load()
    w = _dev(w)
    if w.dtype != torch.float32 or not w.is_contiguous():
        w = w.float().contiguous()
    n, c, k = w.shape
    pn, pc = (c, n) if dgrad else (n, c)
    n_pad, c_pad = round_up(pn, 32), round_up(pc, c_mult)
    out = torch.empty(2 * k * n_pad * c_pad, dtype=torch.float16, device=w.device)
    inv = torch.empty(n_pad, dtype=torch.float32, device=w.device)
    _abi.check(lib.jatts_pack_conv_weight_split(w.data_ptr(), n, c, k, c_mult, int(dgrad), out.data_ptr(), inv.data_ptr(), _stream()),
               "jatts_pack_conv_weight_split")
    return out, inv, c_pad


def convtranspose_as_conv(w, stride, padding):
    c_in, c_out, K = w.shape
    qs = [(r, q) for r in range(stride) for q in range(-K, K + 1) if 0 <= stride * q + r + padding < K]
    qmin, qmax = min(q for _, q in qs), max(q for _, q in qs)
    taps = qmax - qmin + 1
    wc = torch.zeros(stride * c_out, c_in, taps, dtype=w.dtype, device=w.device)
    for r, q in qs:
        kk = stride * q + r + padding
        wc[r * c_out:(r + 1) * c_out, :, qmax - q] = w[:, :, kk].t()
    return wc, qmax


def conv1d(rb, xs, w_packed, c_in, n_out, k_w, *, dtype, dil=1, pad=None, bias=None, act=ACT_NONE,
           alpha=1.0, resid=None, out=None, out_f32=False, transposed=False, pre_lrelu=None,
           in_scale=1.0, ldx=None, x_col0=0, len_mul=1, out_ld=None, out_col0=0, out_rows=None, resid_col0=0,
           y_seq_col0=None, reflect=False, variant=0, w_inv=None, snake=None, split=None, w_layout=0):
    lib = _abi.load()
    if isinstance(xs, torch.Tensor):
        xs = [xs]
    if isinstance(w_packed, SplitWeight):
        if dtype != F32:
            raise ValueError("conv1d: a SplitWeight goes with dtype F32 tensors")
        if (k_w - 1) * dil <= 32:
            dtype, w_inv, w_packed, out_f32 = F32S, w_packed.inv, w_packed.packed, True
        else:
            w_packed = w_packed.f32()
    elif isinstance(w_packed, EmulWeight):
        if dtype != F32:
            raise ValueError("conv1d: an EmulWeight goes with dtype F32 tensors")
        if (k_w - 1) * dil <= 32:
            dtype, w_layout, w_packed, out_f32 = w_packed.code, w_packed.layout, w_packed.packed, True
        else:
            w_packed = w_packed.f32()
    x0 = _dev(xs[0])
    rows = rb.total * len_mul
    tdt = torch_dtype(dtype)
    for x in xs:
        if x.dtype != tdt or not x.is_contiguous():
            raise ValueError(f"conv1d: inputs must be contiguous {tdt}")
    ldx = ldx if ldx is not None else x0.shape[-1]
    if x0.numel() < rows * ldx or max(x_col0 if isinstance(x_col0, (list, tuple)) else [x_col0]) + c_in > ldx:
        raise ValueError("conv1d: input too small for the ragged geometry")
    if pad is None:
        pad = (k_w - 1) // 2 * dil
    n_pad = round_up(n_out, 32)
    if dtype == F32S:
        if w_packed.dtype != torch.float16 or w_packed.numel() != 2 * n_pad * c_in * k_w or w_inv is None or w_inv.numel() != n_pad:
            raise ValueError("conv1d: F32S takes the (packed, inverse scales) pair of pack_conv_weight_split")
    elif dtype in EMUL:
        if w_packed.dtype != torch.bfloat16 or w_packed.numel() != 3 * n_pad * c_in * k_w:
            raise ValueError("conv1d: F32E / F32E6 take the packed bf16 terms of pack_conv_weight_bf16x3")
        out_f32 = True
    elif w_packed.dtype != tdt or w_packed.numel() != n_pad * c_in * k_w:
        raise ValueError("conv1d: packed weight has wrong dtype/size")
    odt = torch.float32 if out_f32 else tdt
    out2 = None
    if split is not None:
        n_split, ld2, col2 = split
        if transposed or out is not None or resid is not None or n_split % 256 or not 0 < n_split < n_out:
            raise ValueError("conv1d: split takes a fresh row-major output, no residual, n_split a multiple of 256 below n_out")
        out = torch.empty(rows, out_ld or n_split, dtype=odt, device=x0.device)
        out2 = torch.empty(n_out - n_split, ld2, dtype=odt, device=x0.device)
    if out is None:
        if transposed:
            out = torch.empty(n_out, rows if out_ld is None else out_ld, dtype=odt, device=x0.device)
        else:
            out = torch.empty(rows if out_rows is None else out_rows, out_ld or n_out, dtype=odt, device=x0.device)
    if out.dtype != odt:
        raise ValueError("conv1d: output dtype mismatch")
    ldy = out.shape[-1] if out_ld is None else out_ld
    d = _abi.ConvDesc()
    d.rg = rb.struct(len_mul)
    d.dtype, d.n_in = dtype, len(xs)
    cols = x_col0 if isinstance(x_col0, (list, tuple)) else [x_col0] * len(xs)
    for i, x in enumerate(xs):
        d.x[i] = _ptr(x, cols[i])
    d.pad_mode = _abi.PAD_REFLECT if reflect else _abi.PAD_ZERO
    d.variant = variant
    d.ldx, d.in_scale = ldx, in_scale
    d.pre_act = _abi.PRE_LRELU if pre_lrelu is not None else _abi.PRE_NONE
    d.pre_slope = pre_lrelu or 0.0
    d.w, d.c_in, d.n_out, d.k_w, d.dil, d.pad = w_packed.data_ptr(), c_in, n_out, k_w, dil, pad
    d.bias = _ptr(bias)
    d.act, d.alpha = act, alpha
    if snake is not None:
        if act != ACT_NONE or any(v.dtype != torch.float32 or v.numel() != n_out or not v.is_contiguous() for v in snake):
            raise ValueError("conv1d: snake takes two contiguous f32 vectors of n_out and replaces act")
        d.act, d.act_a, d.act_b = _abi.ACT_SNAKEBETA, snake[0].data_ptr(), snake[1].data_ptr()
    if resid is not None:
        if resid.dtype != torch.float32:
            raise ValueError("conv1d: residual must be f32")
        d.resid, d.ldr = _ptr(resid, resid_col0), resid.shape[-1]
    d.y, d.ldy = _ptr(out, out_col0), ldy
    d.y_is_f32, d.y_transposed = int(odt == torch.float32), int(transposed)
    d.y_seq_col0 = _ptr(y_seq_col0) if transposed else None
    d.w_inv = _ptr(w_inv) if dtype == F32S else None
    d.w_layout = w_layout if dtype in EMUL else 0
    if out2 is not None:
        d.n_split, d.ldy2, d.y2, d.y2_seq_col0 = split[0], split[1], out2.data_ptr(), _ptr(split[2])
    _count(2.0 * c_in * n_out * k_w * rows)
    with _Timed("conv1d", (c_in, n_out, k_w, rows)):
        _abi.check(lib.jatts_conv1d(C.byref(d), _stream()), "jatts_conv1d")
    return out if out2 is None else (out, out2)


def _check_unit_weights(who, dtype, channels, k_w, *ws):
    n = channels * channels * k_w
    want = {F32: (torch.float32, n), F16: (torch.float16, n), F32S: (torch.float16, 2 * n), F32E: (torch.bfloat16, 3 * n), F32E6: (torch.bfloat16, 3 * n)}[dtype]
    for w in ws:
        if w.dtype != want[0] or w.numel() != want[1] or not w.is_cuda:
            raise ValueError(f"{who}: dtype code {dtype} needs packed weights of {want[1]} x {want[0]} on the GPU (pack_conv_weight / pack_conv_weight_split / "
                             f"pack_conv_weight_bf16x3 with c_mult=32), got {w.numel()} x {w.dtype}")


def hifigan_resunit(rb, len_mul, x, y, w1, b1, w2, b2, channels, k_w, dil, slope, dtype, add=None, out_scale=1.0, ws=None, w_layout=0):
    lib = _abi.load()
    d = _abi.ResUnitDesc()
    d.w_layout = w_layout
    d.rg = rb.struct(len_mul)
    d.dtype, d.channels, d.k_w, d.dil, d.slope = dtype, channels, k_w, dil, slope
    rows = rb.total * len_mul
    if x.numel() != rows * channels or y.numel() != rows * channels or x.dtype != torch_dtype(dtype):
        raise ValueError("hifigan_resunit: bad buffer size/dtype")
    d.x, d.y = _dev(x).data_ptr(), y.data_ptr()
    _check_unit_weights("hifigan_resunit", dtype, channels, k_w, w1, w2)
    d.w1, d.b1, d.w2, d.b2 = w1.data_ptr(), b1.data_ptr(), w2.data_ptr(), b2.data_ptr()
    if dtype == F32S:
        if ws is None or ws[0].numel() < channels or ws[1].numel() < channels or ws[0].dtype != torch.float32:
            raise ValueError("hifigan_resunit: F32S needs the inverse weight scales (pack_conv_weight_split)")
        d.ws1, d.ws2 = ws[0].data_ptr(), ws[1].data_ptr()
    if add:
        for a in add:
            if a.numel() != rows * channels or a.dtype != x.dtype:
                raise ValueError("hifigan_resunit: bad mix buffer")
        d.add0 = add[0].data_ptr()
        d.add1 = add[1].data_ptr() if len(add) > 1 else None
    d.out_scale = out_scale
    with _Timed("resunit", (channels, k_w, dil, rows, len(add) if add else 0)):
        _abi.check(lib.jatts_hifigan_resunit(C.byref(d), _stream()), "jatts_hifigan_resunit")
    return y


def hifigan_resblock(rb, len_mul, x, y, units, channels, k_w, slope, dtype, add=None, out_scale=1.0, ws=None):
    lib = _abi.load()
    d = _abi.ResBlockDesc()
    d.rg = rb.struct(len_mul)
    d.dtype, d.channels, d.k_w, d.n_units, d.slope = dtype, channels, k_w, len(units), slope
    rows = rb.total * len_mul
    if x.numel() != rows * channels or y.numel() != rows * channels or x.dtype != torch_dtype(dtype):
        raise ValueError("hifigan_resblock: bad buffer size/dtype")
    d.x, d.y = _dev(x).data_ptr(), y.data_ptr()
    for i, (w1, b1, w2, b2, dil) in enumerate(units):
        _check_unit_weights("hifigan_resblock", dtype, channels, k_w, w1, w2)
        d.w1[i], d.b1[i], d.w2[i], d.b2[i], d.dil[i] = w1.data_ptr(), b1.data_ptr(), w2.data_ptr(), b2.data_ptr(), dil
    if dtype == F32S:
        if ws is None or len(ws) != len(units):
            raise ValueError("hifigan_resblock: F32S needs the inverse weight scales of every unit")
        for i, (a, b) in enumerate(ws):
            d.ws1[i], d.ws2[i] = a.data_ptr(), b.data_ptr()
    if add:
        for a in add:
            if a.numel() != rows * channels or a.dtype != x.dtype:
                raise ValueError("hifigan_resblock: bad mix buffer")
        d.add0 = add[0].data_ptr()
        d.add1 = add[1].data_ptr() if len(add) > 1 else None
    d.out_scale = out_scale
    with _Timed("resblock", (channels, k_w, tuple(u[4] for u in units), rows, len(add) if add else 0)):
        _abi.check(lib.jatts_hifigan_resblock(C.byref(d), _stream()), "jatts_hifigan_resblock")
    return y


def hifigan_output(rb, len_mul, xs, in_scale, slope, c_in, k_w, w, bias, dtype):
    lib = _abi.load()
    rows = rb.total * len_mul
    y = torch.empty(rows, dtype=torch.float32, device=xs[0].device)
    arr = (C.c_void_p * len(xs))(*[_dev(x).data_ptr() for x in xs])
    rg = rb.struct(len_mul)
    _abi.check(lib.jatts_hifigan_output(C.byref(rg), dtype, arr, len(xs), in_scale, slope, c_in, k_w,
                                        w.data_ptr(), float(bias), y.data_ptr(), _stream()),
               "jatts_hifigan_output")
    return y


def relpos_attention(rb, q, ldq, k, ldk, vt, ldvt, g, ldg, ku, scale, n_heads, d_k, dtype,
                     q_col0=0, k_col0=0, rel_mode=1, rel_center=0, vt_col0=None, kv_len=None):
    lib = _abi.load()
    out = torch.empty(rb.total, n_heads * d_k, dtype=torch_dtype(dtype), device=q.device)
    d = _abi.RelAttnDesc()
    d.rg = rb.struct()
    d.dtype, d.n_heads, d.d_k = dtype, n_heads, d_k
    d.q, d.ldq = _ptr(_dev(q), q_col0), ldq
    d.k, d.ldk = _ptr(k, k_col0), ldk
    d.vt, d.ldvt = vt.data_ptr(), ldvt
    d.g, d.ldg = _ptr(g), ldg
    d.ku = _ptr(ku)
    d.scale = scale
    d.out, d.ldo = out.data_ptr(), n_heads * d_k
    d.rel_mode, d.rel_center = rel_mode, rel_center
    d.vt_col0 = _ptr(vt_col0)
    d.kv_len = _ptr(kv_len)
    with _Timed("relattn", (n_heads, d_k, rb.total, sum(v * v for v in rb.lens))):
        _abi.check(lib.jatts_relpos_attention(C.byref(d), _stream()), "jatts_relpos_attention")
    return out


def rowdot(x, ldx, rows, n_heads, d_k, vec, col0=0):
    lib = _abi.load()
    out = torch.empty(rows, n_heads, dtype=torch.float32, device=x.device)
    _abi.check(lib.jatts_rowdot(code_of(x), _ptr(_dev(x), col0), ldx, rows, n_heads, d_k, vec.data_ptr(),
                                out.data_ptr(), _stream()), "jatts_rowdot")
    return out


_BAD_IDS = {}


def _bad_counter(dev):
    key = dev.index if dev.index is not None else torch.cuda.current_device()
    t = _BAD_IDS.get(key)
    if t is None:
        t = _BAD_IDS[key] = torch.zeros(1, dtype=torch.int64, device=dev)
    return t


def embed_scale(ids, table, scale, n_bad=None):
    lib = _abi.load()
    if n_bad is None:
        n_bad = _bad_counter(_dev(ids).device)
    out = torch.empty(ids.numel(), table.shape[1], dtype=torch.float32, device=ids.device)
    _abi.check(lib.jatts_embed_scale(_dev(ids).data_ptr(), ids.numel(), table.data_ptr(), table.shape[1],
                                     float(scale), out.data_ptr(), table.shape[0], _ptr(n_bad), _stream()), "jatts_embed_scale")
    return out


def check_bad_ids(device):
    t = _BAD_IDS.get(torch.device(device).index if torch.device(device).index is not None else torch.cuda.current_device())
    if t is None:
        return
    n = int(t)
    if n:
        t.zero_()
        raise IndexError(f"index out of range in self ({n} token ids outside the embedding table)")


def bad_ids_async(device):
    dev = torch.device(device)
    t = _BAD_IDS.get(dev.index if dev.index is not None else torch.cuda.current_device())
    if t is None:
        return lambda wait=False: True
    host = torch.zeros(1, dtype=torch.int64).pin_memory()
    host.copy_(t, non_blocking=True)
    t.zero_()
    ev = torch.cuda.Event()
    ev.record()

    def resolve(wait=False):
        if wait:
            ev.synchronize()
        elif not ev.query():
            return False
        if int(host):
            n = int(host)
            host.zero_()
            raise IndexError(f"index out of range in self ({n} token ids outside the embedding table in an earlier training step)")
        return True
    return resolve


def layernorm(x, gamma, beta, out_dtype, eps=1e-12, out=None):
    lib = _abi.load()
    rows, dim = x.shape
    if out is None:
        out = torch.empty(rows, dim, dtype=torch_dtype(out_dtype), device=x.device)
    _abi.check(lib.jatts_layernorm(_dev(x).data_ptr(), code_of(x), dim, out.data_ptr(), out_dtype, dim, rows,
                                   dim, gamma.data_ptr(), beta.data_ptr(), eps, _stream()), "jatts_layernorm")
    return out


def affine_cast(x, out_dtype, scale=None, shift=None, ldy=None, x_col0=0, dim=None, out=None, out_col0=0):
    lib = _abi.load()
    rows, ldx = x.shape
    dim = dim if dim is not None else ldx - x_col0
    fresh = out is None
    if fresh:
        ldy = ldy or dim
        out = torch.empty(rows, ldy, dtype=torch_dtype(out_dtype), device=x.device)
        dim_w = dim
    else:
        ldy, dim_w = out.shape[1], dim
        if out.dtype != torch_dtype(out_dtype) or out.shape[0] != rows or out_col0 + dim > ldy:
            raise ValueError("affine_cast: bad output slice")
    fn = lib.jatts_affine_cast if fresh else lib.jatts_affine_slice
    _abi.check(fn(_ptr(_dev(x), x_col0), ldx, _ptr(out, out_col0), out_dtype, ldy, rows, dim_w,
                  _ptr(scale), _ptr(shift), _stream()), "jatts_affine_cast")
    return out


def glu_dwconv_bn_swish(rb, x, channels, k_w, w_dw, bn_scale, bn_shift, dtype):
    lib = _abi.load()
    y = torch.empty(rb.total, channels, dtype=torch_dtype(dtype), device=x.device)
    rg = rb.struct()
    _abi.check(lib.jatts_glu_dwconv_bn_swish(C.byref(rg), dtype, _dev(x).data_ptr(), y.data_ptr(), channels,
                                             k_w, w_dw.data_ptr(), bn_scale.data_ptr(), bn_shift.data_ptr(),
                                             _stream()), "jatts_glu_dwconv_bn_swish")
    return y


def predictor_head(x, w, b, want_duration=False, offset=1.0):
    lib = _abi.load()
    rows, dim = x.shape
    v = torch.empty(rows, dtype=torch.float32, device=x.device)
    dur = torch.empty(rows, dtype=torch.int64, device=x.device) if want_duration else None
    _abi.check(lib.jatts_predictor_head(code_of(x), _dev(x).data_ptr(), dim, rows, dim, w.data_ptr(), float(b),
                                        v.data_ptr(), _ptr(dur), offset, _stream()), "jatts_predictor_head")
    return (v, dur) if want_duration else v


def variance_embed_add(rb, hs, p, wp, bp, e, we, be):
    lib = _abi.load()
    rg = rb.struct()
    _abi.check(lib.jatts_variance_embed_add(C.byref(rg), _dev(hs).data_ptr(), hs.shape[1], p.data_ptr(),
                                            wp.data_ptr(), bp.data_ptr(), wp.shape[-1], e.data_ptr(),
                                            we.data_ptr(), be.data_ptr(), we.shape[-1], _stream()),
               "jatts_variance_embed_add")
    return hs


def gated_tanh_sigmoid(rb, x, gseq, channels, dtype):
    lib = _abi.load()
    y = torch.empty(rb.total, channels, dtype=torch_dtype(dtype), device=x.device)
    rg = rb.struct()
    _abi.check(lib.jatts_gated_tanh_sigmoid(C.byref(rg), dtype, _dev(x).data_ptr(), _ptr(gseq), y.data_ptr(),
                                            channels, _stream()), "jatts_gated_tanh_sigmoid")
    return y


def groupnorm_mish(rb, x, channels, groups, gamma, beta, out_dtype, eps=1e-5, addvec=None, time_split=True):
    lib = _abi.load()
    y = torch.empty(rb.total, channels, dtype=torch_dtype(out_dtype), device=x.device)
    rg = rb.struct()
    ws = None
    if time_split:
        ws = torch.empty(rb.n_seq * groups * ((rb.max_len + 63) // 64) * 3, dtype=torch.float32, device=x.device)
    _abi.check(lib.jatts_groupnorm_mish(C.byref(rg), _dev(x).data_ptr(), code_of(x), y.data_ptr(), out_dtype, channels,
                                        groups, gamma.data_ptr(), beta.data_ptr(), eps, _ptr(addvec), _ptr(ws), _stream()),
               "jatts_groupnorm_mish")
    return y


def snakebeta(x, alpha, inv_beta):
    lib = _abi.load()
    y = torch.empty_like(x)
    _abi.check(lib.jatts_snakebeta(code_of(x), _dev(x).data_ptr(), y.data_ptr(), x.shape[0], x.shape[1],
                                   alpha.data_ptr(), inv_beta.data_ptr(), _stream()), "jatts_snakebeta")
    return y


def l2_normalize(x, out_dtype, ldy=None, eps=1e-12):
    lib = _abi.load()
    rows, dim = x.shape
    ldy = ldy or dim
    y = torch.empty(rows, ldy, dtype=torch_dtype(out_dtype), device=x.device)
    _abi.check(lib.jatts_l2_normalize(_dev(x).data_ptr(), dim, y.data_ptr(), out_dtype, ldy, rows, dim, eps,
                                      _stream()), "jatts_l2_normalize")
    return y


def gaussian_sample(stats, noise, noise_scale):
    lib = _abi.load()
    rows, c2 = stats.shape
    z = torch.empty(rows, c2 // 2, dtype=torch.float32, device=stats.device)
    _abi.check(lib.jatts_gaussian_sample(_dev(stats).data_ptr(), noise.data_ptr(), z.data_ptr(), rows, c2 // 2,
                                         float(noise_scale), _stream()), "jatts_gaussian_sample")
    return z


def flip_channels(x):
    lib = _abi.load()
    y = torch.empty_like(x)
    _abi.check(lib.jatts_flip_channels(_dev(x).data_ptr(), y.data_ptr(), x.shape[0], x.shape[1], _stream()),
               "jatts_flip_channels")
    return y


def add_seq_vector(rb, hs, vec):
    lib = _abi.load()
    rg = rb.struct()
    _abi.check(lib.jatts_add_seq_vector(C.byref(rg), _dev(hs).data_ptr(), hs.shape[1], vec.data_ptr(),
                                        _stream()), "jatts_add_seq_vector")
    return hs


def lr_durations(rb, d, alpha=1.0, zero_rule=2):
    lib = _abi.load()
    d_eff = torch.empty_like(d)
    cum = torch.empty_like(d)
    buf = torch.empty(2 * rb.n_seq, dtype=torch.int64, device=d.device)
    rg = rb.struct()
    _abi.check(lib.jatts_lr_durations(C.byref(rg), _dev(d).data_ptr(), float(alpha), int(zero_rule),
                                      d_eff.data_ptr(), cum.data_ptr(), buf.data_ptr(), _stream()),
               "jatts_lr_durations")
    return d_eff, cum, buf[:rb.n_seq], (buf[rb.n_seq:] if zero_rule == 2 else None)


def lr_sizes_dev(rb, d, alpha=1.0, check=None):
    d_eff, cum, olens, fb = lr_durations(rb, d, alpha)
    return d_eff, cum, torch.cat([olens, fb] + ([check.view(-1)] if check is not None else []))


def lr_sizes_host(rb, sizes, checked):
    host = sizes.tolist()
    if checked and host[2 * rb.n_seq]:
        raise IndexError("token id out of range")
    olens_h, fb_h = host[:rb.n_seq], host[rb.n_seq:2 * rb.n_seq]
    if any(fb_h):
        import logging
        logging.warning("predicted durations includes all 0 sequences. fill the first element with 1.")
    return olens_h


def lr_sizes(rb, d, alpha=1.0, check=None):
    d_eff, cum, sizes = lr_sizes_dev(rb, d, alpha, check)
    return d_eff, cum, lr_sizes_host(rb, sizes, check is not None)


def zero_pad_rows(rb, x, valid_len, len_mul=1):
    lib = _abi.load()
    dim = x.shape[1] if x.dim() == 2 else 1
    rg = rb.struct(len_mul)
    _abi.check(lib.jatts_zero_pad_rows(C.byref(rg), _dev(x).data_ptr(), code_of(x), dim, dim, valid_len.data_ptr(), _stream()),
               "jatts_zero_pad_rows")
    return x


def cfm_mix(rb, x1, z, t, sigma_min):
    lib = _abi.load()
    y, u = torch.empty_like(x1), torch.empty_like(x1)
    rg = rb.struct()
    _abi.check(lib.jatts_cfm_mix(C.byref(rg), _dev(x1).data_ptr(), z.data_ptr(), t.data_ptr(), float(sigma_min), x1.shape[1],
                                 y.data_ptr(), u.data_ptr(), _stream()), "jatts_cfm_mix")
    return y, u


def sq_err_sum(a, b, scale=1.0):
    lib = _abi.load()
    out = torch.empty((), dtype=torch.float32, device=a.device)
    ws = torch.empty(256, dtype=torch.float64, device=a.device)
    _abi.check(lib.jatts_sq_err_sum(_dev(a).data_ptr(), b.data_ptr(), a.numel(), float(scale), out.data_ptr(), ws.data_ptr(),
                                    _stream()), "jatts_sq_err_sum")
    return out


def lr_gather(rb_in, cum, rb_out, x, want_index=False):
    lib = _abi.load()
    dim = x.shape[1]
    out = torch.empty(rb_out.total, dim, dtype=torch.float32, device=x.device)
    idx = torch.empty(rb_out.total, dtype=torch.int64, device=x.device) if want_index else None
    rg = rb_in.struct()
    _abi.check(lib.jatts_lr_gather(C.byref(rg), cum.data_ptr(), rb_out.cu.data_ptr(), rb_out.max_len,
                                   _dev(x).data_ptr(), dim, out.data_ptr(), _ptr(idx), _stream()),
               "jatts_lr_gather")
    return (out, idx) if want_index else out


def gaussian_upsample(rb_in, d, rb_out, hs, delta=0.1):
    lib = _abi.load()
    dim = hs.shape[1]
    out = torch.empty(rb_out.total, dim, dtype=torch.float32, device=hs.device)
    rg = rb_in.struct()
    _abi.check(lib.jatts_gaussian_upsample(C.byref(rg), _dev(d).data_ptr(), rb_out.cu.data_ptr(),
                                           rb_out.max_len, hs.data_ptr(), dim, delta, out.data_ptr(),
                                           _stream()), "jatts_gaussian_upsample")
    return out


def alignment_logp(rb_f, rb_t, feats, text, adim):
    lib = _abi.load()
    ld = round_up(max(rb_t.max_len, 1), 8)
    out = torch.empty(rb_f.total, ld, dtype=torch.float32, device=feats.device)
    rg = rb_f.struct()
    _abi.check(lib.jatts_alignment_logp(C.byref(rg), rb_t.cu.data_ptr(), rb_t.max_len, _dev(feats).data_ptr(),
                                        _dev(text).data_ptr(), adim, out.data_ptr(), ld, _stream()), "jatts_alignment_logp")
    return out


def mas_viterbi(rb_f, rb_t, log_p):
    lib = _abi.load()
    dev = log_p.device
    path = torch.empty(rb_f.total, dtype=torch.int64, device=dev)
    dur = torch.empty(rb_t.total, dtype=torch.int64, device=dev)
    score = torch.empty(rb_f.n_seq, dtype=torch.float64, device=dev)
    rg = rb_f.struct()
    if log_p.dtype != torch.float32 or not log_p.is_contiguous():
        raise ValueError("mas_viterbi: log_p must be contiguous float32")
    _abi.check(lib.jatts_mas_viterbi(C.byref(rg), rb_t.cu.data_ptr(), _dev(log_p).data_ptr(), log_p.shape[1], rb_t.max_len,
                                     path.data_ptr(), dur.data_ptr(), score.data_ptr(), _stream()), "jatts_mas_viterbi")
    return path, dur, score


def pcm16(y, out=None):
    lib = _abi.load()
    y = _dev(y)
    if y.dtype != torch.float32 or not y.is_contiguous():
        raise ValueError("pcm16: contiguous float32 expected")
    if out is None:
        out = torch.empty(y.numel(), dtype=torch.int16, device=y.device)
    _abi.check(lib.jatts_pcm16(y.data_ptr(), y.numel(), out.data_ptr(), _stream()), "jatts_pcm16")
    return out


def frame_signal(rb_frames, cu_samples, x, window, n_fft, hop, ldo):
    lib = _abi.load()
    out = torch.empty(rb_frames.total, ldo, dtype=torch.float32, device=x.device)
    rg = rb_frames.struct()
    _abi.check(lib.jatts_frame_signal(C.byref(rg), cu_samples.data_ptr(), _dev(x).data_ptr(), window.data_ptr(), n_fft, hop,
                                      out.data_ptr(), ldo, _stream()), "jatts_frame_signal")
    return out


def power_spectrum(x, n_bins, ldo):
    lib = _abi.load()
    out = torch.empty(x.shape[0], ldo, dtype=torch.float32, device=x.device)
    _abi.check(lib.jatts_power_spectrum(_dev(x).data_ptr(), x.shape[1], n_bins, x.shape[0], out.data_ptr(), ldo, _stream()),
               "jatts_power_spectrum")
    return out


def fbank_post(rb, p, n_mels, ldo, amin=1e-10, top_db=80.0):
    lib = _abi.load()
    out = torch.empty(rb.total, ldo, dtype=torch.float32, device=p.device)
    rg = rb.struct()
    _abi.check(lib.jatts_fbank_post(C.byref(rg), _dev(p).data_ptr(), p.shape[1], n_mels, amin, top_db, out.data_ptr(), ldo,
                                    _stream()), "jatts_fbank_post")
    return out


def seq_mean_std(rb, x, dim, logits=None, want_std=True, eps=1e-12):
    lib = _abi.load()
    ld = 2 * dim if want_std else dim
    out = torch.empty(rb.n_seq, ld, dtype=torch.float32, device=x.device)
    rg = rb.struct()
    _abi.check(lib.jatts_seq_mean_std(C.byref(rg), _dev(x).data_ptr(), x.shape[1], dim, _ptr(logits),
                                      logits.shape[1] if logits is not None else 0, out.data_ptr(),
                                      _ptr(out, dim) if want_std else None, ld, eps, _stream()), "jatts_seq_mean_std")
    return out


def seq_affine_act(rb, x, dim, out_dtype, seq_vec=None, pre_act=ACT_NONE, scale=None, shift=None, post_act=ACT_NONE, ldy=None):
    lib = _abi.load()
    ldy = ldy or dim
    y = torch.empty(rb.total, ldy, dtype=torch_dtype(out_dtype), device=x.device)
    rg = rb.struct()
    _abi.check(lib.jatts_seq_affine_act(C.byref(rg), _dev(x).data_ptr(), x.shape[1], dim, _ptr(seq_vec), pre_act, _ptr(scale),
                                        _ptr(shift), post_act, y.data_ptr(), out_dtype, ldy, _stream()), "jatts_seq_affine_act")
    return y


def se_scale_add(rb, x, s, resid=None, out=None, out_col0=0):
    lib = _abi.load()
    y = torch.empty_like(x) if out is None else out
    rg = rb.struct()
    _abi.check(lib.jatts_se_scale_add(C.byref(rg), _dev(x).data_ptr(), x.shape[1], s.data_ptr(), _ptr(resid), _ptr(y, out_col0),
                                      y.shape[1], _stream()), "jatts_se_scale_add")
    return y


def masked_loss(rb, a, b, valid_len, kind, scale, log_offset=-1.0):
    lib = _abi.load()
    a2 = a if a.dim() == 2 else a.reshape(-1, 1)
    b2 = b if b.dim() == 2 else b.reshape(-1, 1)
    out = torch.empty((), dtype=torch.float32, device=a.device)
    ws = torch.empty(4 * rb.n_seq, dtype=torch.float64, device=a.device)
    rg = rb.struct()
    _abi.check(lib.jatts_masked_loss(C.byref(rg), _dev(a2).data_ptr(), a2.shape[1], b2.data_ptr(), b2.shape[1], a2.shape[1],
                                     _ptr(valid_len), kind, float(log_offset), float(scale), out.data_ptr(), ws.data_ptr(), _stream()),
               "jatts_masked_loss")
    return out


def conv1d_wgrad(rb, x, dy, c_in, n_out, k_w, dil, pad, len_mul=1, want_db=False):
    lib = _abi.load()
    dw = torch.empty(n_out, c_in, k_w, dtype=torch.float32, device=x.device)
    db = torch.empty(n_out, dtype=torch.float32, device=x.device) if want_db else None
    ws = torch.empty(rb.n_seq * (k_w * round_up(n_out, 64) * round_up(c_in, 64) + round_up(n_out, 64)), dtype=torch.float32,
                     device=x.device)
    rg = rb.struct(len_mul)
    _count(2.0 * c_in * n_out * k_w * rb.total * len_mul)
    _ws(x.device)
    _ws_check(lib.jatts_conv1d_wgrad(C.byref(rg), _dev(x).data_ptr(), x.shape[1], dy.data_ptr(), dy.shape[1], c_in, n_out, k_w, dil,
                                      pad, dw.data_ptr(), _ptr(db), ws.data_ptr(), _stream()), "jatts_conv1d_wgrad")
    return (dw, db) if want_db else dw


def col_sum(x, dim=None):
    lib = _abi.load()
    dim = dim or x.shape[1]
    out = _zeros((dim), x.device)
    _ws(x.device)
    _ws_check(lib.jatts_col_sum(_dev(x).data_ptr(), x.shape[1], x.shape[0], dim, out.data_ptr(), _stream()), "jatts_col_sum")
    return out


ACT_MODE = {"relu": 1, "tanh": 2, "swish": 3, "mish": 4}


def _f32c(t):
    t = _dev(t)
    if t.dtype != torch.float32 or not t.is_contiguous():
        raise ValueError("training ops take contiguous f32 device tensors")
    return t


def layernorm_bwd(x, dy, gamma, eps, need_dx=True, need_dparam=True):
    lib = _abi.load()
    x, dy = _f32c(x), _f32c(dy)
    rows, dim = x.shape
    dx = torch.empty_like(x) if need_dx else None
    dg = _zeros((dim), x.device) if need_dparam else None
    db = _zeros((dim), x.device) if need_dparam else None
    _ws(x.device)
    _ws_check(lib.jatts_layernorm_bwd(x.data_ptr(), dim, dy.data_ptr(), dim, _f32c(gamma).data_ptr(), rows, dim, float(eps), _ptr(dx), dim,
                                       _ptr(dg), _ptr(db), _stream()), "jatts_layernorm_bwd")
    return dx, dg, db


def act_fwd(x, mode):
    lib = _abi.load()
    x = _f32c(x)
    y = torch.empty_like(x)
    _abi.check(lib.jatts_act_fwd(ACT_MODE[mode], x.data_ptr(), y.data_ptr(), x.numel(), _stream()), "jatts_act_fwd")
    return y


def act_bwd(x, dy, mode):
    lib = _abi.load()
    x, dy = _f32c(x), _f32c(dy)
    dx = torch.empty_like(x)
    _abi.check(lib.jatts_act_bwd(ACT_MODE[mode], x.data_ptr(), dy.data_ptr(), dx.data_ptr(), x.numel(), _stream()), "jatts_act_bwd")
    return dx


def glu_fwd(x):
    lib = _abi.load()
    x = _f32c(x)
    rows, c2 = x.shape
    y = torch.empty(rows, c2 // 2, dtype=torch.float32, device=x.device)
    _abi.check(lib.jatts_glu_fwd(x.data_ptr(), y.data_ptr(), rows, c2 // 2, _stream()), "jatts_glu_fwd")
    return y


def glu_bwd(x, dy):
    lib = _abi.load()
    x, dy = _f32c(x), _f32c(dy)
    dx = torch.empty_like(x)
    _abi.check(lib.jatts_glu_bwd(x.data_ptr(), dy.data_ptr(), dx.data_ptr(), x.shape[0], x.shape[1] // 2, _stream()), "jatts_glu_bwd")
    return dx


def dwconv(rb, x, w, bias, pad, flip=False):
    lib = _abi.load()
    x, w = _f32c(x), _f32c(w)
    y = torch.empty_like(x)
    rg = rb.struct()
    _abi.check(lib.jatts_dwconv(C.byref(rg), x.data_ptr(), w.data_ptr(), _ptr(bias), y.data_ptr(), x.shape[1], w.shape[1], pad, int(flip),
                                _stream()), "jatts_dwconv")
    return y


def dwconv_wgrad(rb, x, dy, k_w, pad):
    lib = _abi.load()
    x, dy = _f32c(x), _f32c(dy)
    dw = _zeros((x.shape[1], k_w), x.device)
    rg = rb.struct()
    _ws(x.device)
    _ws_check(lib.jatts_dwconv_wgrad(C.byref(rg), x.data_ptr(), dy.data_ptr(), dw.data_ptr(), x.shape[1], k_w, pad, _stream()),
               "jatts_dwconv_wgrad")
    return dw


def col_stats(x, y2=None, shift=None, mul=None):
    lib = _abi.load()
    x = _f32c(x)
    rows, dim = x.shape
    o0 = _zeros((dim), x.device)
    o1 = _zeros((dim), x.device)
    _ws(x.device)
    _ws_check(lib.jatts_col_stats(x.data_ptr(), _ptr(y2), dim, rows, dim, _ptr(shift), _ptr(mul), 0 if y2 is None else 1, o0.data_ptr(),
                                   o1.data_ptr(), _stream()), "jatts_col_stats")
    return o0, o1


def bn_bwd_apply(x, dy, mean, rstd, gamma, s_dy, s_dyx):
    lib = _abi.load()
    x, dy = _f32c(x), _f32c(dy)
    dx = torch.empty_like(x)
    _abi.check(lib.jatts_bn_bwd_apply(x.data_ptr(), dy.data_ptr(), x.shape[0], x.shape[1], mean.data_ptr(), rstd.data_ptr(),
                                      _f32c(gamma).data_ptr(), s_dy.data_ptr(), s_dyx.data_ptr(), dx.data_ptr(), _stream()), "jatts_bn_bwd_apply")
    return dx


def index_add_rows(src, idx, n_dst, scale=1.0, skip=-1):
    lib = _abi.load()
    src = _f32c(src)
    dst = _zeros((n_dst, src.shape[1]), src.device)
    _abi.check(lib.jatts_index_add_rows(src.data_ptr(), src.shape[1], _dev(idx).data_ptr(), src.shape[0], src.shape[1], float(scale), int(skip),
                                        n_dst, dst.data_ptr(), _stream()), "jatts_index_add_rows")
    return dst


def lr_segment_sum(rb_in, cum, rb_out, dy):
    lib = _abi.load()
    dy = _f32c(dy)
    dhs = torch.empty(rb_in.total, dy.shape[1], dtype=torch.float32, device=dy.device)
    rg = rb_in.struct()
    _abi.check(lib.jatts_lr_segment_sum(C.byref(rg), _dev(cum).data_ptr(), rb_out.cu.data_ptr(), dy.data_ptr(), dy.shape[1], dhs.data_ptr(),
                                        _stream()), "jatts_lr_segment_sum")
    return dhs


def shift_softmax_fwd(ac, bd, lens, scale, mode=1):
    lib = _abi.load()
    ac = _f32c(ac)
    B, H, T, _ = ac.shape
    p = torch.empty_like(ac)
    _abi.check(lib.jatts_shift_softmax_fwd(ac.data_ptr(), _ptr(bd), B, H, T, _ptr(lens), float(scale), mode, p.data_ptr(), _stream()),
               "jatts_shift_softmax_fwd")
    return p


def shift_softmax_bwd(p, dp, scale, need_dbd=True, mode=1):
    lib = _abi.load()
    p, dp = _f32c(p), _f32c(dp)
    B, H, T, _ = p.shape
    ds = torch.empty_like(p)
    dbd = torch.empty(B, H, T, 2 * T - 1 if mode == 2 else T, dtype=torch.float32, device=p.device) if need_dbd else None
    _abi.check(lib.jatts_shift_softmax_bwd(p.data_ptr(), dp.data_ptr(), B, H, T, float(scale), mode, ds.data_ptr(), _ptr(dbd), _stream()),
               "jatts_shift_softmax_bwd")
    return ds, dbd


def gate_bwd(x, dy):
    lib = _abi.load()
    x, dy = _f32c(x), _f32c(dy)
    dx = torch.empty_like(x)
    _abi.check(lib.jatts_gate_bwd(x.data_ptr(), dy.data_ptr(), dx.data_ptr(), x.shape[0], x.shape[1] // 2, _stream()), "jatts_gate_bwd")
    return dx


def weight_norm_fwd(v, g):
    lib = _abi.load()
    v, g = _f32c(v), _f32c(g)
    n_out = v.shape[0]
    w = torch.empty_like(v)
    inv = torch.empty(n_out, dtype=torch.float32, device=v.device)
    _abi.check(lib.jatts_weight_norm_fwd(v.data_ptr(), g.data_ptr(), n_out, v.numel() // n_out, w.data_ptr(), inv.data_ptr(), _stream()),
               "jatts_weight_norm_fwd")
    return w, inv


def weight_norm_bwd(v, g, inv, dw):
    lib = _abi.load()
    v, g, dw = _f32c(v), _f32c(g), _f32c(dw)
    n_out = v.shape[0]
    dv, dg = torch.empty_like(v), torch.empty_like(g)
    _abi.check(lib.jatts_weight_norm_bwd(v.data_ptr(), g.data_ptr(), inv.data_ptr(), dw.data_ptr(), n_out, v.numel() // n_out,
                                         dv.data_ptr(), dg.data_ptr(), _stream()), "jatts_weight_norm_bwd")
    return dv, dg


def split_add(o, h, skip=None):
    lib = _abi.load()
    o, h = _f32c(o), _f32c(h)
    rows, dim = h.shape
    if o.shape != (rows, 2 * dim):
        raise ValueError("split_add: o must be (rows, 2 dim)")
    h_out, s_out = torch.empty_like(h), torch.empty_like(h)
    _abi.check(lib.jatts_split_add(o.data_ptr(), h.data_ptr(), _ptr(_f32c(skip) if skip is not None else None), rows, dim,
                                   h_out.data_ptr(), s_out.data_ptr(), _stream()), "jatts_split_add")
    return h_out, s_out


def concat2(a, b, rows, dim, device):
    lib = _abi.load()
    out = torch.empty(rows, 2 * dim, dtype=torch.float32, device=device)
    _abi.check(lib.jatts_concat2(_ptr(_f32c(a) if a is not None else None), _ptr(_f32c(b) if b is not None else None), rows, dim,
                                 out.data_ptr(), _stream()), "jatts_concat2")
    return out


def outer_rows(v, w, bias=None, out=None):
    lib = _abi.load()
    v, w = _f32c(v), _f32c(w)
    acc = out is not None
    if out is None:
        out = torch.empty(v.numel(), w.numel(), dtype=torch.float32, device=v.device)
    _abi.check(lib.jatts_outer_rows(v.data_ptr(), w.data_ptr(), _ptr(bias), v.numel(), w.numel(), int(acc), out.data_ptr(), _stream()),
               "jatts_outer_rows")
    return out


def col_wsum(x, v):
    lib = _abi.load()
    x, v = _f32c(x), _f32c(v)
    out = _zeros((x.shape[1]), x.device)
    _ws(x.device)
    _ws_check(lib.jatts_col_wsum(x.data_ptr(), x.shape[1], v.data_ptr(), x.shape[0], x.shape[1], out.data_ptr(), _stream()), "jatts_col_wsum")
    return out


def row_dot(x, w, bias=None):
    lib = _abi.load()
    x, w = _f32c(x), _f32c(w)
    y = torch.empty(x.shape[0], dtype=torch.float32, device=x.device)
    _abi.check(lib.jatts_row_dot(x.data_ptr(), x.shape[1], w.data_ptr(), _ptr(bias), x.shape[0], x.shape[1], y.data_ptr(), _stream()),
               "jatts_row_dot")
    return y


def masked_loss_bwd(rb, a, b, valid_len, kind, scale, upstream=None, log_offset=-1.0):
    lib = _abi.load()
    a2 = _f32c(a if a.dim() == 2 else a.reshape(-1, 1))
    b2 = _f32c(b if b.dim() == 2 else b.reshape(-1, 1))
    da = torch.empty_like(a2)
    rg = rb.struct()
    _abi.check(lib.jatts_masked_loss_bwd(C.byref(rg), a2.data_ptr(), a2.shape[1], b2.data_ptr(), b2.shape[1], a2.shape[1], _ptr(valid_len), kind,
                                         float(log_offset), float(scale), _ptr(upstream), da.data_ptr(), a2.shape[1], _stream()),
               "jatts_masked_loss_bwd")
    return da.view_as(a)


def dropout(x, p, seed, seed_dev=None):
    lib = _abi.load()
    x = _f32c(x)
    y = torch.empty_like(x)
    _abi.check(lib.jatts_dropout(x.data_ptr(), y.data_ptr(), x.numel(), float(p), int(seed) & 0xFFFFFFFFFFFFFFFF, _ptr(seed_dev), _stream()),
               "jatts_dropout")
    return y


def qkv_split(qkv, u, v, B, T, H):
    lib = _abi.load()
    qkv = _f32c(qkv)
    A3 = qkv.shape[1]
    dk = A3 // 3 // H
    if qkv.shape[0] != B * T or dk * H * 3 != A3 or (u is None) != (v is None):
        raise ValueError("qkv_split: shapes")
    if u is not None:
        u, v = _f32c(u), _f32c(v)
        if u.numel() != H * dk or v.numel() != H * dk:
            raise ValueError("qkv_split: bias shapes")
    outs = [torch.empty(B, H, T, dk, dtype=torch.float32, device=qkv.device) for _ in range(4 if u is not None else 3)]
    qu, qv, k, vv = outs if u is not None else (outs[0], None, outs[1], outs[2])
    _abi.check(lib.jatts_qkv_split(qkv.data_ptr(), _ptr(u), _ptr(v), B, T, H, dk, qu.data_ptr(), _ptr(qv), k.data_ptr(), vv.data_ptr(), _stream()),
               "jatts_qkv_split")
    return outs


def qkv_split_bwd(dqu, dqv, dk_, dvv):
    lib = _abi.load()
    dqu, dk_, dvv = _f32c(dqu), _f32c(dk_), _f32c(dvv)
    B, H, T, dk = dqu.shape
    dqkv = torch.empty(B * T, 3 * H * dk, dtype=torch.float32, device=dqu.device)
    du = dv = None
    if dqv is not None:
        dqv = _f32c(dqv)
        du, dv = _zeros((H * dk), dqu.device), _zeros((H * dk), dqu.device)
    _ws(dqu.device)
    _ws_check(lib.jatts_qkv_split_bwd(dqu.data_ptr(), _ptr(dqv), dk_.data_ptr(), dvv.data_ptr(), B, T, H, dk, dqkv.data_ptr(), _ptr(du), _ptr(dv),
                                       _stream()), "jatts_qkv_split_bwd")
    return dqkv, du, dv


def act_dropout(x, mode, p, seed, seed_dev=None, dy=None):
    lib = _abi.load()
    x = _f32c(x)
    out = torch.empty_like(x)
    _abi.check(lib.jatts_act_dropout(ACT_MODE[mode], x.data_ptr(), _ptr(_f32c(dy) if dy is not None else None), out.data_ptr(), x.numel(),
                                     float(p), int(seed) & 0xFFFFFFFFFFFFFFFF, _ptr(seed_dev), _stream()), "jatts_act_dropout")
    return out


def dropout_add(x, resid, p, alpha, seed, seed_dev=None):
    lib = _abi.load()
    x = _f32c(x)
    if resid is not None:
        resid = _f32c(resid)
        if resid.shape != x.shape:
            raise ValueError("dropout_add: shape mismatch")
    y = torch.empty_like(x)
    _abi.check(lib.jatts_dropout_add(x.data_ptr(), _ptr(resid), y.data_ptr(), x.numel(), float(p), float(alpha),
                                     int(seed) & 0xFFFFFFFFFFFFFFFF, _ptr(seed_dev), _stream()), "jatts_dropout_add")
    return y


def sumsq(x, out):
    lib = _abi.load()
    x = _f32c(x)
    _ws(x.device)
    _ws_check(lib.jatts_sumsq(x.data_ptr(), x.numel(), out.data_ptr(), _stream()), "jatts_sumsq")
    return out


def gather_grads(grads, offsets, flat, accumulate=False):
    lib = _abi.load()
    n = len(grads)
    if n == 0:
        return
    for g in grads:
        if g.dtype != torch.float32 or not g.is_contiguous() or g.device != flat.device:
            raise ValueError("gather_grads takes contiguous f32 tensors on the flat buffer's device")
    src = (C.c_void_p * n)(*[g.data_ptr() for g in grads])
    num = (C.c_int64 * n)(*[g.numel() for g in grads])
    off = (C.c_int64 * n)(*[int(o) for o in offsets])
    _abi.check(lib.jatts_gather_grads(src, num, off, n, flat.data_ptr(), 1 if accumulate else 0, _stream()), "jatts_gather_grads")


def adam_hyper(lr, beta1, beta2, eps, weight_decay, step):
    bc1, bc2 = 1.0 - beta1 ** step, 1.0 - beta2 ** step
    return [lr / bc1, 1.0 - beta1, beta2, 1.0 - beta2, eps, weight_decay, bc2 ** 0.5]


def adam_step(p, g, m, v, lr, beta1, beta2, eps, weight_decay, step, grad_sumsq=None, max_norm=0.0, hyper_dev=None):
    lib = _abi.load()
    _abi.check(lib.jatts_adam_step(_f32c(p).data_ptr(), _f32c(g).data_ptr(), _f32c(m).data_ptr(), _f32c(v).data_ptr(), p.numel(), float(lr),
                                   float(beta1), float(beta2), float(eps), float(weight_decay), int(step), _ptr(grad_sumsq), float(max_norm),
                                   _ptr(hyper_dev), _stream()), "jatts_adam_step")


def groupnorm_fwd(rb, x, groups, gamma, beta, eps):
    lib = _abi.load()
    x = _f32c(x)
    y = torch.empty_like(x)
    mean = torch.empty(rb.n_seq * groups, dtype=torch.float32, device=x.device)
    rstd = torch.empty_like(mean)
    rg = rb.struct()
    _abi.check(lib.jatts_groupnorm_fwd(C.byref(rg), x.data_ptr(), x.shape[1], groups, _f32c(gamma).data_ptr(), _f32c(beta).data_ptr(), float(eps),
                                       y.data_ptr(), mean.data_ptr(), rstd.data_ptr(), _stream()), "jatts_groupnorm_fwd")
    return y, mean, rstd


def groupnorm_bwd(rb, x, dy, groups, gamma, mean, rstd, need_dx=True, need_dparam=True):
    lib = _abi.load()
    x, dy = _f32c(x), _f32c(dy)
    dim = x.shape[1]
    dx = torch.empty_like(x) if need_dx else None
    dg = _zeros((dim), x.device) if need_dparam else None
    db = _zeros((dim), x.device) if need_dparam else None
    rg = rb.struct()
    _ws(x.device)
    _ws_check(lib.jatts_groupnorm_bwd(C.byref(rg), x.data_ptr(), dy.data_ptr(), dim, groups, _f32c(gamma).data_ptr(), mean.data_ptr(),
                                       rstd.data_ptr(), _ptr(dx), _ptr(dg), _ptr(db), _stream()), "jatts_groupnorm_bwd")
    return dx, dg, db


def snakebeta_fwd(x, alpha, beta):
    lib = _abi.load()
    x = _f32c(x)
    y = torch.empty_like(x)
    _abi.check(lib.jatts_snakebeta_fwd(x.data_ptr(), y.data_ptr(), x.shape[0], x.shape[1], _f32c(alpha).data_ptr(), _f32c(beta).data_ptr(),
                                       _stream()), "jatts_snakebeta_fwd")
    return y


def snakebeta_bwd(x, dy, alpha, beta):
    lib = _abi.load()
    x, dy = _f32c(x), _f32c(dy)
    dx = torch.empty_like(x)
    da = _zeros((x.shape[1]), x.device)
    db = _zeros((x.shape[1]), x.device)
    _ws(x.device)
    _ws_check(lib.jatts_snakebeta_bwd(x.data_ptr(), dy.data_ptr(), x.shape[0], x.shape[1], _f32c(alpha).data_ptr(), _f32c(beta).data_ptr(),
                                       dx.data_ptr(), da.data_ptr(), db.data_ptr(), _stream()), "jatts_snakebeta_bwd")
    return dx, da, db


def ctc_forward_sum(log_p, ilens, olens, log_blank, want_grad=True, grad_scale=1.0):
    lib = _abi.load()
    log_p = _f32c(log_p)
    B, T, ld = log_p.shape
    max_i = int(ilens.max())
    ws = torch.empty(2 * B * T * (2 * max_i + 1), dtype=torch.float32, device=log_p.device)
    nll = torch.empty(B, dtype=torch.float32, device=log_p.device)
    grad = torch.empty_like(log_p) if want_grad else None
    _up = lambda t: t.to(torch.int32).contiguous() if t.is_cuda else h2d([int(v) for v in t.tolist()], torch.int32, log_p.device)
    il, ol = _up(ilens), _up(olens)
    _abi.check(lib.jatts_ctc_forward_sum(log_p.data_ptr(), B, T, ld, il.data_ptr(), ol.data_ptr(), max_i, float(log_blank), ws.data_ptr(),
                                         nll.data_ptr(), _ptr(grad), float(grad_scale), _stream()), "jatts_ctc_forward_sum")
    return nll, grad


def seq_sum(rb, x):
    lib = _abi.load()
    x = _f32c(x)
    out = _zeros((rb.n_seq, x.shape[1]), x.device)
    rg = rb.struct()
    _ws(x.device)
    _ws_check(lib.jatts_seq_sum(C.byref(rg), x.data_ptr(), x.shape[1], out.data_ptr(), _stream()), "jatts_seq_sum")
    return out


def bgemm(a, b, trans_a=False, trans_b=False, alpha=1.0, out=None):
    lib = _abi.load()
    a, b = _dev(a), _dev(b)

    def geom(t):
        if t.dtype != torch.float32 or t.dim() not in (3, 4) or t.stride(-1) != 1:
            raise ValueError("bgemm: f32 tensors of 3 / 4 dims with contiguous rows")
        if t.dim() == 3:
            return None, t.shape[0], 0, t.stride(0), t.stride(1)
        return t.shape[0], t.shape[1], t.stride(0), t.stride(1), t.stride(2)
    ao, ai, sao, sai, lda = geom(a)
    bo, bi, sbo, sbi, ldb = geom(b)
    O = ao if ao is not None else bo
    if O is None:
        O = 1
    if ai != bi or (ao is not None and ao != O) or (bo is not None and bo != O):
        raise ValueError("bgemm: batch dims differ")
    m, k = (a.shape[-1], a.shape[-2]) if trans_a else (a.shape[-2], a.shape[-1])
    n, kb = (b.shape[-2], b.shape[-1]) if trans_b else (b.shape[-1], b.shape[-2])
    if k != kb:
        raise ValueError("bgemm: contraction sizes differ")
    if out is None:
        out = torch.empty(O, ai, m, n, dtype=torch.float32, device=a.device)
    elif (not out.is_cuda or out.dtype != torch.float32 or out.dim() != 4 or tuple(out.shape) != (O, ai, m, n) or out.stride(3) != 1
          or out.device != a.device):
        raise ValueError(f"bgemm: out must be an f32 device tensor of shape {(O, ai, m, n)} with contiguous rows")
    _count(2.0 * O * ai * m * n * k)
    with _Timed("bgemm", (O * ai, m, n, k)):
        _abi.check(lib.jatts_bgemm(a.data_ptr(), sao, sai, lda, int(trans_a), b.data_ptr(), sbo, sbi, ldb, int(trans_b), out.data_ptr(), out.stride(0),
                                   out.stride(1), out.stride(2), O, ai, m, n, k, float(alpha), 0, _stream()), "jatts_bgemm")
    return out


def mfma_ceiling(dtype=F32E, feed=1, target_ms=60.0, device=None, seed=0):
    lib = _abi.load()
    dev = torch.device(device) if device is not None else torch.device("cuda", torch.cuda.current_device())
    g = torch.Generator().manual_seed(seed)
    v = torch.randn(1 << 16, generator=g)
    if dtype in EMUL or dtype == 16 + F32E:
        ops = torch.cat([t.reshape(-1) for t in bf16x3_terms(v)])
    elif dtype in (F16, F32S, 16 + F16):
        ops = v.half()
    else:
        ops = v
    ops = ops.to(dev).contiguous()
    clocks = torch.zeros(2, dtype=torch.int64, device=dev)
    sink = torch.zeros(1, dtype=torch.float32, device=dev)
    wgs = 2 * torch.cuda.get_device_properties(dev).multi_processor_count

    def run(iters):
        a, b = torch.cuda.Event(enable_timing=True), torch.cuda.Event(enable_timing=True)
        a.record()
        _abi.check(lib.jatts_mfma_probe(dtype, feed, ops.data_ptr(), ops.numel() * ops.element_size(), iters, wgs, clocks.data_ptr(), sink.data_ptr(),
                                        _stream()), "jatts_mfma_probe")
        b.record()
        b.synchronize()
        return a.elapsed_time(b)

    it = 2000
    ms = run(it)
    it = max(2000, min(int(it * target_ms / max(ms, 1e-3)) & ~1, 1 << 24))
    run(it)
    ms = run(it)
    c = clocks.tolist()
    return dict(tflops=lib.jatts_mfma_probe_flops(dtype, it, wgs) / ms / 1e9, ms=ms, clock_ghz=c[0] / (c[1] * 10.0) if c[1] else None, iters=it, workgroups=wgs,
                feed="lds" if feed else "registers")


_MARKER = {}


def mfma_marker(device=None):
    lib = _abi.load()
    dev = torch.device(device) if device is not None else torch.device("cuda", torch.cuda.current_device())
    key = str(dev)
    if key not in _MARKER:
        _MARKER[key] = (torch.zeros(1 << 15, dtype=torch.bfloat16, device=dev), torch.zeros(1, dtype=torch.float32, device=dev))
    ops, sink = _MARKER[key]
    _abi.check(lib.jatts_mfma_probe(F32E, 0, ops.data_ptr(), ops.numel() * 2, 2, 1, None, sink.data_ptr(), _stream()), "jatts_mfma_probe")
```

Measured before the change: 64.57 million samples/s.

## Add persistent sliding-window variant to emulated HiFi-GAN resunit kernel

Adds a SLIDE variant of the bf16x3 resunit kernel. It launches one persistent workgroup per CU×occupancy slot, and each workgroup walks a contiguous range of frames across sequences. After the first tile, the halo from the previous tile is kept in a small LDS tail region, so later tiles emit a full WGCOLS outputs without recomputing the halo columns. This aims to cut redundant halo loads and compute, plus launch overhead from many small tiles. The costs are extra LDS, serial tiles per workgroup that may hurt load balance, and an auto-pick heuristic that only applies to non-RREG configs with enough positions.

Result: faster. 66.79 million samples/s, median of 6 (+3.4%).

```diff
diff --git a/include/jatts_hip.h b/include/jatts_hip.h
--- a/include/jatts_hip.h
+++ b/include/jatts_hip.h
@@ -7,7 +7,7 @@
 extern "C" {
 #endif
 
-#define JATTS_ABI_VERSION 4
+#define JATTS_ABI_VERSION 5
 
 #define JATTS_F32 0
 #define JATTS_F16 1
@@ -106,9 +106,12 @@
   const float* ws1;
   const float* ws2;
   int32_t w_layout;
+  int32_t variant;
 } jatts_resunit_desc;
 
 int jatts_hifigan_resunit(const jatts_resunit_desc* d, void* stream);
+
+int jatts_resunit_variant(const jatts_resunit_desc* d);
 
 int64_t jatts_unit_weight_index_k32(int32_t n, int32_t tap, int32_t c, int32_t channels);
 
diff --git a/jatts_amd/_abi.py b/jatts_amd/_abi.py
--- a/jatts_amd/_abi.py
+++ b/jatts_amd/_abi.py
@@ -5,7 +5,7 @@
 LIB_PATH = os.environ.get("JATTS_HIP_LIB") or os.path.join(_HERE, "lib", "libjatts_hip.so")
 
 F32, F16, F32S, F32E, F32E6 = 0, 1, 2, 3, 4
-ABI_VERSION = 4
+ABI_VERSION = 5
 ACT_NONE, ACT_RELU, ACT_TANH, ACT_SWISH, ACT_MISH, ACT_SNAKEBETA = 0, 1, 2, 3, 4, 5
 PRE_NONE, PRE_LRELU = 0, 1
 PAD_ZERO, PAD_REFLECT = 0, 1
@@ -35,7 +35,7 @@
         ("dil", C.c_int32), ("slope", C.c_float), ("x", C.c_void_p), ("y", C.c_void_p),
         ("w1", C.c_void_p), ("b1", C.c_void_p), ("w2", C.c_void_p), ("b2", C.c_void_p),
         ("add0", C.c_void_p), ("add1", C.c_void_p), ("out_scale", C.c_float),
-        ("ws1", C.c_void_p), ("ws2", C.c_void_p), ("w_layout", C.c_int32),
+        ("ws1", C.c_void_p), ("ws2", C.c_void_p), ("w_layout", C.c_int32), ("variant", C.c_int32),
     ]
 
 
@@ -66,6 +66,7 @@
     "jatts_conv1d": (C.c_int, [C.POINTER(ConvDesc), C.c_void_p]),
     "jatts_conv_weight_index": (C.c_int64, [C.c_int32] * 5),
     "jatts_hifigan_resunit": (C.c_int, [C.POINTER(ResUnitDesc), C.c_void_p]),
+    "jatts_resunit_variant": (C.c_int, [C.POINTER(ResUnitDesc)]),
     "jatts_unit_weight_index_k32": (C.c_int64, [C.c_int32] * 4),
     "jatts_hifigan_resblock": (C.c_int, [C.POINTER(ResBlockDesc), C.c_void_p]),
     "jatts_debug_trace": (C.c_int, [C.c_void_p, C.c_int64]),
diff --git a/jatts_amd/csrc/conv_api.hip b/jatts_amd/csrc/conv_api.hip
--- a/jatts_amd/csrc/conv_api.hip
+++ b/jatts_amd/csrc/conv_api.hip
@@ -13,7 +13,7 @@
 int jatts_resunit_f16_wide(const jatts_resunit_desc& d, hipStream_t s);
 int jatts_resunit_f32(const jatts_resunit_desc& d, hipStream_t s);
 int jatts_resunit_split(const jatts_resunit_desc& d, hipStream_t s);
-int jatts_resunit_emul(const jatts_resunit_desc& d, hipStream_t s);
+int jatts_resunit_emul(const jatts_resunit_desc& d, hipStream_t s, int* pick);
 int jatts_resblock_f16(const jatts_resblock_desc& d, hipStream_t s);
 int jatts_resblock_f32(const jatts_resblock_desc& d, hipStream_t s);
 int jatts_resblock_split(const jatts_resblock_desc& d, hipStream_t s);
@@ -67,12 +67,17 @@
   return jatts_set_error_msg(JATTS_ERR_ARG, "conv1d: unknown dtype");
 }
 
-extern "C" int jatts_hifigan_resunit(const jatts_resunit_desc* d, void* stream) {
+static int resunit_check(const jatts_resunit_desc* d) {
   if (!d || !d->x || !d->y || !d->w1 || !d->w2 || !d->b1 || !d->b2 || !d->rg.cu_rows)
     return jatts_set_error_msg(JATTS_ERR_ARG, "resunit: null pointer");
   if (d->x == d->y) return jatts_set_error_msg(JATTS_ERR_ARG, "resunit: y must not alias x");
   if (d->k_w < 1 || !(d->k_w & 1) || d->dil < 1) return jatts_set_error_msg(JATTS_ERR_ARG, "resunit: odd k_w and dil>=1 required");
   if (!(d->slope >= 0.f && d->slope <= 1.f)) return jatts_set_error_msg(JATTS_ERR_ARG, "resunit: LeakyReLU slope must be in [0, 1]");
+  return JATTS_OK;
+}
+
+extern "C" int jatts_hifigan_resunit(const jatts_resunit_desc* d, void* stream) {
+  if (const int rc = resunit_check(d)) return rc;
   if (d->rg.max_len <= 0) return JATTS_OK;
   hipStream_t s = (hipStream_t)stream;
   if (d->dtype == JATTS_F16) return d->channels <= 64 ? jatts_resunit_f16_narrow(*d, s) : jatts_resunit_f16_wide(*d, s);
@@ -83,10 +88,20 @@
   }
   if (d->dtype == JATTS_F32E || d->dtype == JATTS_F32E6) {
     if (d->w_layout != 0 && d->w_layout != 1) return jatts_set_error_msg(JATTS_ERR_ARG, "resunit: w_layout must be 0 or 1");
-    return jatts_resunit_emul(*d, s);
+    return jatts_resunit_emul(*d, s, nullptr);
   }
   if (d->w_layout != 0) return jatts_set_error_msg(JATTS_ERR_ARG, "resunit: w_layout = 1 goes with JATTS_F32E / JATTS_F32E6 only");
   return jatts_set_error_msg(JATTS_ERR_UNSUPPORTED, "resunit: unsupported channels/dtype (use jatts_conv1d)");
+}
+
+extern "C" int jatts_resunit_variant(const jatts_resunit_desc* d) {
+  if (const int rc = resunit_check(d)) return rc;
+  int form = 1;
+  if (d->rg.max_len > 0 && (d->dtype == JATTS_F32E || d->dtype == JATTS_F32E6)) {
+    if (d->w_layout != 0 && d->w_layout != 1) return jatts_set_error_msg(JATTS_ERR_ARG, "resunit: w_layout must be 0 or 1");
+    if (const int rc = jatts_resunit_emul(*d, nullptr, &form)) return rc;
+  }
+  return form;
 }
 
 extern "C" int jatts_hifigan_resblock(const jatts_resblock_desc* d, void* stream) {
diff --git a/jatts_amd/csrc/resunit_emul.hip b/jatts_amd/csrc/resunit_emul.hip
--- a/jatts_amd/csrc/resunit_emul.hip
+++ b/jatts_amd/csrc/resunit_emul.hip
@@ -22,22 +22,26 @@
 }
 
 template <typename T>
-static int resunit_emul16(const jatts_resunit_desc& d, hipStream_t s) {
+static int resunit_emul16(const jatts_resunit_desc& d, hipStream_t s, int* pick) {
   const int halo = (d.k_w - 1) * d.dil;
   switch (d.channels) {
-    case 32: return launch_resunit_emul16<T, 32, 256, 1, 4, 2, false, true>(d, s);
+    case 32: return launch_resunit_emul16<T, 32, 256, 1, 4, 2, false, true>(d, s, pick);
     case 64:
-      if (d.k_w >= 11) return launch_resunit_emul16<T, 64, 256, 1, 4, 1, false, true>(d, s);
-      return launch_resunit_emul16<T, 64, 128, 2, 2, 2, false, true>(d, s);
-    case 128: return launch_resunit_emul16<T, 128, 128, 2, 2, 1>(d, s);
+      if (d.k_w >= 11) return launch_resunit_emul16<T, 64, 256, 1, 4, 1, false, true>(d, s, pick);
+      return launch_resunit_emul16<T, 64, 128, 2, 2, 2, false, true>(d, s, pick);
+    case 128: return launch_resunit_emul16<T, 128, 128, 2, 2, 1>(d, s, pick);
     case 256:
-      if ((64 + halo) * 1552 + 2048 <= 160 * 1024) return launch_resunit_emul16<T, 256, 64, 4, 1, 1>(d, s);
-      return launch_resunit_emul16<T, 256, 64, 4, 1, 1, true>(d, s);
+      if ((64 + halo) * 1552 + 2048 <= 160 * 1024) return launch_resunit_emul16<T, 256, 64, 4, 1, 1>(d, s, pick);
+      return launch_resunit_emul16<T, 256, 64, 4, 1, 1, true>(d, s, pick);
   }
   return jatts_set_error_msg(JATTS_ERR_UNSUPPORTED, "resunit: unsupported channels for JATTS_F32E (32 / 64 / 128 / 256)");
 }
 
-int jatts_resunit_emul(const jatts_resunit_desc& d, hipStream_t s) {
-  if (d.w_layout == 1) return d.dtype == JATTS_F32E6 ? resunit_emul16<bf3f>(d, s) : resunit_emul16<bf3>(d, s);
+int jatts_resunit_emul(const jatts_resunit_desc& d, hipStream_t s, int* pick) {
+  if (d.w_layout == 1) return d.dtype == JATTS_F32E6 ? resunit_emul16<bf3f>(d, s, pick) : resunit_emul16<bf3>(d, s, pick);
+  if (pick) {
+    *pick = 1;
+    return JATTS_OK;
+  }
   return d.dtype == JATTS_F32E6 ? resunit_emul<bf3f>(d, s) : resunit_emul<bf3>(d, s);
 }
diff --git a/jatts_amd/csrc/resunit_emul16_impl.h b/jatts_amd/csrc/resunit_emul16_impl.h
--- a/jatts_amd/csrc/resunit_emul16_impl.h
+++ b/jatts_amd/csrc/resunit_emul16_impl.h
@@ -149,7 +149,7 @@
   }
 }
 
-template <typename T, int C, int WGCOLS, int WN, int WT, int OCC, bool KSPLIT = false, bool RREG = false>
+template <typename T, int C, int WGCOLS, int WN, int WT, int OCC, bool KSPLIT = false, bool RREG = false, bool SLIDE = false>
 __global__ __launch_bounds__(WN* WT * 64, OCC) void resunit_emul16_kernel(jatts_resunit_desc d, unsigned long long* trace, unsigned trace_cap,
                                                                          unsigned bias_off) {
   typedef typename Elem<T>::vec8 V8;
@@ -158,6 +158,7 @@
   constexpr int KC32 = C / 32, NFR16 = C / 16;
   constexpr int pitch = C * 6 + 16;
   constexpr int pitch_x = KSPLIT ? (C / 2) * 6 + 16 : pitch;
+  constexpr int pitch_t = C * 6;
   constexpr int NTHR = WN * WT * 64;
   static_assert(NF * WN * 16 == C && NT * WT * 16 == WGCOLS && C % 32 == 0, "tile shape");
   static_assert(sizeof(T) == 6, "bf3 is three packed bf16");
@@ -180,13 +181,24 @@
   const int p2 = (K - 1) / 2, p1 = p2 * dil;
   const int tt_out = WGCOLS - 2 * p2;
 
-  int b = blockIdx.y, bx = blockIdx.x;
-  if (ragged_is_1d(d.rg) && !ragged_locate(d.rg, tt_out, blockIdx.x, b, bx)) return;
-  const int row_b = d.rg.cu_rows[b];
-  const int L = (d.rg.cu_rows[b + 1] - row_b) * d.rg.len_mul;
-  const int t0 = bx * tt_out;
-  if (t0 >= L) return;
-  const int64_t seq_row0 = (int64_t)row_b * d.rg.len_mul;
+  int b, t0;
+  int64_t f_seq = 0, f_end = 0;
+  if constexpr (!SLIDE) {
+    int bx = blockIdx.x;
+    b = blockIdx.y;
+    if (ragged_is_1d(d.rg) && !ragged_locate(d.rg, tt_out, blockIdx.x, b, bx)) return;
+    t0 = bx * tt_out;
+  } else {
+    const int c0 = d.rg.cu_rows[0];
+    const int64_t total = (int64_t)(d.rg.cu_rows[d.rg.n_seq] - c0) * d.rg.len_mul;
+    const int64_t per = (total + gridDim.x - 1) / gridDim.x;
+    const int64_t f = (int64_t)blockIdx.x * per;
+    if (f >= total) return;
+    f_end = min(total, f + per);
+    b = find_seq(d.rg.cu_rows, d.rg.n_seq, c0 + (int)(f / d.rg.len_mul));
+    f_seq = (int64_t)(d.rg.cu_rows[b] - c0) * d.rg.len_mul;
+    t0 = (int)(f - f_seq);
+  }
   const int lane = threadIdx.x & 63, wave = threadIdx.x >> 6;
   const int wn = wave / WT, wt = wave % WT;
   const int g4 = lane >> 4;
@@ -197,12 +209,10 @@
   char* xs = smem;
   char* hs = smem;
   float* bs = reinterpret_cast<float*>(smem + bias_off);
+  char* tl = smem + bias_off - (SLIDE ? (K - 1) * pitch_t : 0);
   for (int u = threadIdx.x; u < 2 * C; u += NTHR) bs[u] = u < C ? d.b1[u] : d.b2[u - C];
 
   WStream16<T, NF> ws;
-  ws.bind((const T*)d.w1, KC32, NFR16, nf0, lane);
-  ws.fetch(0, 0);
-
   typename Acc16<T>::type acc[NF][NT];
   auto bias_acc = [&](const float* bv) {
 #pragma unroll
@@ -227,233 +237,301 @@
     return o;
   };
   const float* x = (const float*)d.x;
-  const int pos0 = t0 - p2 - p1;
-  if constexpr (!KSPLIT) {
-    constexpr int UPR = C / 8;
-    constexpr int UB = 8;
-    const int total = rx * UPR;
-    if constexpr (RREG) {
-      const int r_in = p1 + p2, n_in = tt_out * UPR;
-#pragma unroll
-      for (int j = 0; j < MAXI; ++j) {
-        const int v = threadIdx.x + j * NTHR;
-        const int ro = v / UPR, cu = v - ro * UPR;
-        const int pos = t0 + ro;
-        if (v < n_in && pos < L) xk[j] = Vec8IO<float>::ldg(x + (seq_row0 + pos) * (int64_t)C + cu * 8);
-        else xk[j] = f32x8{0, 0, 0, 0, 0, 0, 0, 0};
-      }
-      const int n_halo = (rx - tt_out) * UPR;
-      for (int base = threadIdx.x; base < n_halo; base += NTHR * UB) {
-        f32x8 v[UB];
-#pragma unroll
-        for (int j = 0; j < UB; ++j) {
-          const int u = base + j * NTHR;
-          int r = u / UPR;
-          const int cu = u - r * UPR;
-          if (r >= r_in) r += tt_out;
-          const int pos = pos0 + r;
-          if (u < n_halo && pos >= 0 && pos < L) v[j] = Vec8IO<float>::ldg(x + (seq_row0 + pos) * (int64_t)C + cu * 8);
-          else v[j] = f32x8{0, 0, 0, 0, 0, 0, 0, 0};
-        }
-#pragma unroll
-        for (int j = 0; j < UB; ++j) {
-          const int u = base + j * NTHR;
-          if (u >= n_halo) continue;
-          int r = u / UPR;
-          const int cu = u - r * UPR;
-          if (r >= r_in) r += tt_out;
-          Vec8IO<T>::sts(xs + (size_t)r * pitch + (size_t)cu * 48, to_planes(v[j]));
-        }
-      }
-#pragma unroll
-      for (int j = 0; j < MAXI; ++j) {
-        const int v = threadIdx.x + j * NTHR;
-        if (v >= n_in) continue;
-        const int ro = v / UPR, cu = v - ro * UPR;
-        Vec8IO<T>::sts(xs + (size_t)(r_in + ro) * pitch + (size_t)cu * 48, to_planes(xk[j]));
-      }
+  bool slide = false;
+  for (bool first = true;; first = false) {
+    unsigned tid = threadIdx.x;
+    if constexpr (SLIDE) asm volatile("" : "+v"(tid));
+    const int row_b = d.rg.cu_rows[b];
+    const int L = (d.rg.cu_rows[b + 1] - row_b) * d.rg.len_mul;
+    if constexpr (!SLIDE) {
+      if (t0 >= L) return;
+    }
+    const int64_t seq_row0 = (int64_t)row_b * d.rg.len_mul;
+    const int off = slide ? 2 * p2 : 0;
+    const int nout = slide ? WGCOLS : tt_out;
+    int nvalid = min(nout, L - t0);
+    if constexpr (SLIDE) {
+      nvalid = (int)min((int64_t)nvalid, f_end - f_seq - t0);
+      if (!first) __syncthreads();
+    }
+
+    ws.bind((const T*)d.w1, KC32, NFR16, nf0, lane);
+    ws.fetch(0, 0);
+    const int pos0 = t0 - p2 + off - p1;
+    if constexpr (!KSPLIT) {
+      constexpr int UPR = C / 8;
+      constexpr int UB = 8;
+      const int total = rx * UPR;
+      if constexpr (RREG) {
+        const int r_in = p1 + p2 - off, n_in = nout * UPR;
+#pragma unroll
+        for (int j = 0; j < MAXI; ++j) {
+          const int v = tid + j * NTHR;
+          const int ro = v / UPR, cu = v - ro * UPR;
+          const int pos = t0 + ro;
+          if (v < n_in && pos < L) xk[j] = Vec8IO<float>::ldg(x + (seq_row0 + pos) * (int64_t)C + cu * 8);
+          else xk[j] = f32x8{0, 0, 0, 0, 0, 0, 0, 0};
+        }
+        const int n_halo = (rx - nout) * UPR;
+        for (int base = tid; base < n_halo; base += NTHR * UB) {
+          f32x8 v[UB];
+#pragma unroll
+          for (int j = 0; j < UB; ++j) {
+            const int u = base + j * NTHR;
+            int r = u / UPR;
+            const int cu = u - r * UPR;
+            if (r >= r_in) r += nout;
+            const int pos = pos0 + r;
+            if (u < n_halo && pos >= 0 && pos < L) v[j] = Vec8IO<float>::ldg(x + (seq_row0 + pos) * (int64_t)C + cu * 8);
+            else v[j] = f32x8{0, 0, 0, 0, 0, 0, 0, 0};
+          }
+#pragma unroll
+          for (int j = 0; j < UB; ++j) {
+            const int u = base + j * NTHR;
+            if (u >= n_halo) continue;
+            int r = u / UPR;
+            const int cu = u - r * UPR;
+            if (r >= r_in) r += nout;
+            Vec8IO<T>::sts(xs + (size_t)r * pitch + (size_t)cu * 48, to_planes(v[j]));
+          }
+        }
+#pragma unroll
+        for (int j = 0; j < MAXI; ++j) {
+          const int v = tid + j * NTHR;
+          if (v >= n_in) continue;
+          const int ro = v / UPR, cu = v - ro * UPR;
+          Vec8IO<T>::sts(xs + (size_t)(r_in + ro) * pitch + (size_t)cu * 48, to_planes(xk[j]));
+        }
+      } else {
+        constexpr int UBX = ((WGCOLS + 64) * UPR + NTHR - 1) / NTHR;
+        for (int base = tid; base < total; base += NTHR * UBX) {
+          f32x8 v[UBX];
+#pragma unroll
+          for (int j = 0; j < UBX; ++j) {
+            const int u = base + j * NTHR;
+            const int r = u / UPR, cu = u - r * UPR;
+            const int pos = pos0 + r;
+            if (u < total && pos >= 0 && pos < L) v[j] = Vec8IO<float>::ldg(x + (seq_row0 + pos) * (int64_t)C + cu * 8);
+            else v[j] = f32x8{0, 0, 0, 0, 0, 0, 0, 0};
+          }
+#pragma unroll
+          for (int j = 0; j < UBX; ++j) {
+            const int u = base + j * NTHR;
+            if (u >= total) continue;
+            const int r = u / UPR, cu = u - r * UPR;
+            Vec8IO<T>::sts(xs + (size_t)r * pitch + (size_t)cu * 48, to_planes(v[j]));
+          }
+        }
+      }
+      __syncthreads();
+      JATTS_STAMP(2);
+      bias_acc(bs);
+      conv16<T, NF, NT, KC32>(acc, ws, 0, K, dil, xs, pitch, col0, lane, (const T*)d.w2 + (size_t)nf0 * 512 + (size_t)lane * 8);
     } else {
-      constexpr int UBX = ((WGCOLS + 64) * UPR + NTHR - 1) / NTHR;
-      for (int base = threadIdx.x; base < total; base += NTHR * UBX) {
-        f32x8 v[UBX];
-#pragma unroll
-        for (int j = 0; j < UBX; ++j) {
-          const int u = base + j * NTHR;
+      constexpr int UPR = C / 16;
+      constexpr int MAXU = ((WGCOLS + 64) * UPR + NTHR - 1) / NTHR;
+      const int total = rx * UPR;
+      f32x8 xv[MAXU];
+      auto load_half = [&](int half) {
+#pragma unroll
+        for (int j = 0; j < MAXU; ++j) {
+          const int u = tid + j * NTHR;
           const int r = u / UPR, cu = u - r * UPR;
           const int pos = pos0 + r;
-          if (u < total && pos >= 0 && pos < L) v[j] = Vec8IO<float>::ldg(x + (seq_row0 + pos) * (int64_t)C + cu * 8);
-          else v[j] = f32x8{0, 0, 0, 0, 0, 0, 0, 0};
-        }
-#pragma unroll
-        for (int j = 0; j < UBX; ++j) {
-          const int u = base + j * NTHR;
-          if (u >= total) continue;
-          const int r = u / UPR, cu = u - r * UPR;
-          Vec8IO<T>::sts(xs + (size_t)r * pitch + (size_t)cu * 48, to_planes(v[j]));
-        }
-      }
-    }
+          if (u < total && pos >= 0 && pos < L) xv[j] = Vec8IO<float>::ldg(x + (seq_row0 + pos) * (int64_t)C + half * (C / 2) + cu * 8);
+          else xv[j] = f32x8{0, 0, 0, 0, 0, 0, 0, 0};
+        }
+      };
+      auto store_half = [&]() {
+#pragma unroll
+        for (int j = 0; j < MAXU; ++j) {
+          const int u = tid + j * NTHR;
+          if (u < total) Vec8IO<T>::sts(xs + (size_t)(u / UPR) * pitch_x + (size_t)(u % UPR) * 48, to_planes(xv[j]));
+        }
+      };
+      load_half(0);
+      store_half();
+      load_half(1);
+      __syncthreads();
+      JATTS_STAMP(2);
+      bias_acc(bs);
+      conv16<T, NF, NT, KC32 / 2>(acc, ws, 0, K, dil, xs, pitch_x, col0, lane, ws.wl + (size_t)(KC32 / 2) * ws.kc_stride);
+      lds_barrier();
+      store_half();
+      lds_barrier();
+      conv16<T, NF, NT, KC32 / 2>(acc, ws, KC32 / 2, K, dil, xs, pitch_x, col0, lane, (const T*)d.w2 + (size_t)nf0 * 512 + (size_t)lane * 8);
+    }
+    finish_acc();
+    JATTS_STAMP(3);
+
+    lds_barrier();
+    JATTS_STAMP(10);
+    if (SLIDE && slide) {
+      for (int u = tid; u < (K - 1) * (C / 8); u += NTHR) {
+        const int r = u / (C / 8), cu = u % (C / 8);
+        Vec8IO<T>::sts(hs + (size_t)r * pitch + (size_t)cu * 48, Vec8IO<T>::lds(tl + (size_t)r * pitch_t + (size_t)cu * 48));
+      }
+    } else {
+      for (int u = tid; u < (K - 1) * (C / 8); u += NTHR) {
+        const int r = WGCOLS + u / (C / 8), cu = u % (C / 8);
+        V8 z;
+#pragma unroll
+        for (int e = 0; e < 8; ++e) z.b0[e] = z.b1[e] = z.b2[e] = (bf16)0.f;
+        Vec8IO<T>::sts(hs + (size_t)r * pitch + (size_t)cu * 48, z);
+      }
+    }
+#pragma unroll
+    for (int t = 0; t < NT; ++t) {
+      const int col = col0 + t * 16 + (lane & 15);
+      const int pos = t0 - p2 + off + col;
+      const float keep = (pos >= 0 && pos < L) ? 1.f : 0.f;
+#pragma unroll
+      for (int f = 0; f < NF; ++f) {
+        const int n0 = (nf0 + f) * 16 + 4 * g4;
+        float v[4];
+#pragma unroll
+        for (int e = 0; e < 4; ++e) {
+          const float a = acc16_val(acc[f][t])[e] * keep;
+          v[e] = fmaxf(a, a * d.slope);
+        }
+        bf16x4 q0, q1, q2;
+        bf3_split4(v, q0, q1, q2);
+        char* p = hs + (size_t)(col + off) * pitch + (size_t)(n0 >> 3) * 48 + (size_t)(n0 & 4) * 2;
+        *reinterpret_cast<bf16x4*>(p) = q0;
+        *reinterpret_cast<bf16x4*>(p + 16) = q1;
+        *reinterpret_cast<bf16x4*>(p + 32) = q2;
+      }
+    }
+    JATTS_STAMP(12);
+    lds_barrier();
+    JATTS_STAMP(4);
+
+    bias_acc(bs + C);
+    ws.bind((const T*)d.w2, KC32, NFR16, nf0, lane);
+    conv16<T, NF, NT, KC32>(acc, ws, 0, K, 1, hs, pitch, col0, lane, nullptr);
+    finish_acc();
+    JATTS_STAMP(5);
+
     __syncthreads();
-    JATTS_STAMP(2);
-    bias_acc(bs);
-    conv16<T, NF, NT, KC32>(acc, ws, 0, K, dil, xs, pitch, col0, lane, (const T*)d.w2 + (size_t)nf0 * 512 + (size_t)lane * 8);
-  } else {
-    constexpr int UPR = C / 16;
-    constexpr int MAXU = ((WGCOLS + 64) * UPR + NTHR - 1) / NTHR;
-    const int total = rx * UPR;
-    f32x8 xv[MAXU];
-    auto load_half = [&](int half) {
-#pragma unroll
-      for (int j = 0; j < MAXU; ++j) {
-        const int u = threadIdx.x + j * NTHR;
-        const int r = u / UPR, cu = u - r * UPR;
-        const int pos = pos0 + r;
-        if (u < total && pos >= 0 && pos < L) xv[j] = Vec8IO<float>::ldg(x + (seq_row0 + pos) * (int64_t)C + half * (C / 2) + cu * 8);
-        else xv[j] = f32x8{0, 0, 0, 0, 0, 0, 0, 0};
-      }
-    };
-    auto store_half = [&]() {
-#pragma unroll
-      for (int j = 0; j < MAXU; ++j) {
-        const int u = threadIdx.x + j * NTHR;
-        if (u < total) Vec8IO<T>::sts(xs + (size_t)(u / UPR) * pitch_x + (size_t)(u % UPR) * 48, to_planes(xv[j]));
-      }
-    };
-    load_half(0);
-    store_half();
-    load_half(1);
+    if constexpr (SLIDE) {
+      for (int u = tid; u < (K - 1) * (C / 8); u += NTHR) {
+        const int r = u / (C / 8), cu = u % (C / 8);
+        Vec8IO<T>::sts(tl + (size_t)r * pitch_t + (size_t)cu * 48, Vec8IO<T>::lds(hs + (size_t)(nout + r) * pitch + (size_t)cu * 48));
+      }
+    }
+    char* ys = smem;
+#pragma unroll
+    for (int t = 0; t < NT; ++t) {
+      const int col = col0 + t * 16 + (lane & 15);
+      if (col >= nvalid) continue;
+#pragma unroll
+      for (int f = 0; f < NF; ++f) {
+        const int n0 = (nf0 + f) * 16 + 4 * g4;
+        *reinterpret_cast<f32x4*>(ys + (size_t)col * pitch + (size_t)n0 * 4) = acc16_val(acc[f][t]);
+      }
+    }
     __syncthreads();
-    JATTS_STAMP(2);
-    bias_acc(bs);
-    conv16<T, NF, NT, KC32 / 2>(acc, ws, 0, K, dil, xs, pitch_x, col0, lane, ws.wl + (size_t)(KC32 / 2) * ws.kc_stride);
-    lds_barrier();
-    store_half();
-    lds_barrier();
-    conv16<T, NF, NT, KC32 / 2>(acc, ws, KC32 / 2, K, dil, xs, pitch_x, col0, lane, (const T*)d.w2 + (size_t)nf0 * 512 + (size_t)lane * 8);
-  }
-  finish_acc();
-  JATTS_STAMP(3);
-
-  lds_barrier();
-  JATTS_STAMP(10);
-  for (int u = threadIdx.x; u < (K - 1) * (C / 8); u += NTHR) {
-    const int r = WGCOLS + u / (C / 8), cu = u % (C / 8);
-    V8 z;
-#pragma unroll
-    for (int e = 0; e < 8; ++e) z.b0[e] = z.b1[e] = z.b2[e] = (bf16)0.f;
-    Vec8IO<T>::sts(hs + (size_t)r * pitch + (size_t)cu * 48, z);
-  }
-#pragma unroll
-  for (int t = 0; t < NT; ++t) {
-    const int col = col0 + t * 16 + (lane & 15);
-    const int pos = t0 - p2 + col;
-    const float keep = (pos >= 0 && pos < L) ? 1.f : 0.f;
-#pragma unroll
-    for (int f = 0; f < NF; ++f) {
-      const int n0 = (nf0 + f) * 16 + 4 * g4;
-      float v[4];
-#pragma unroll
-      for (int e = 0; e < 4; ++e) {
-        const float a = acc16_val(acc[f][t])[e] * keep;
-        v[e] = fmaxf(a, a * d.slope);
-      }
-      bf16x4 q0, q1, q2;
-      bf3_split4(v, q0, q1, q2);
-      char* p = hs + (size_t)col * pitch + (size_t)(n0 >> 3) * 48 + (size_t)(n0 & 4) * 2;
-      *reinterpret_cast<bf16x4*>(p) = q0;
-      *reinterpret_cast<bf16x4*>(p + 16) = q1;
-      *reinterpret_cast<bf16x4*>(p + 32) = q2;
-    }
-  }
-  JATTS_STAMP(12);
-  lds_barrier();
-  JATTS_STAMP(4);
-
-  bias_acc(bs + C);
-  ws.bind((const T*)d.w2, KC32, NFR16, nf0, lane);
-  conv16<T, NF, NT, KC32>(acc, ws, 0, K, 1, hs, pitch, col0, lane, nullptr);
-  finish_acc();
-  JATTS_STAMP(5);
-
-  __syncthreads();
-  char* ys = smem;
-#pragma unroll
-  for (int t = 0; t < NT; ++t) {
-    const int col = col0 + t * 16 + (lane & 15);
-    if (col >= tt_out || t0 + col >= L) continue;
-#pragma unroll
-    for (int f = 0; f < NF; ++f) {
-      const int n0 = (nf0 + f) * 16 + 4 * g4;
-      *reinterpret_cast<f32x4*>(ys + (size_t)col * pitch + (size_t)n0 * 4) = acc16_val(acc[f][t]);
-    }
-  }
-  __syncthreads();
-  JATTS_STAMP(6);
-  {
-    const int vrows = min(tt_out, L - t0);
-    const int64_t g0 = (seq_row0 + t0) * (int64_t)C;
-    constexpr bool keep_small = C <= 64;
-    const float* xg = (const float*)d.x;
-    float* yg = (float*)d.y;
-    if constexpr (RREG) {
-      constexpr int UPR = C / 8;
-      const int n_out = vrows * UPR;
-      const bool has_add1 = d.add0 != nullptr && d.add1 != nullptr;
-      f32x8 a0[MAXI], a1[MAXI];
-      if (d.add0) {
+    JATTS_STAMP(6);
+    {
+      const int vrows = nvalid;
+      const int64_t g0 = (seq_row0 + t0) * (int64_t)C;
+      constexpr bool keep_small = C <= 64;
+      const float* xg = (const float*)d.x;
+      float* yg = (float*)d.y;
+      if constexpr (RREG) {
+        constexpr int UPR = C / 8;
+        const int n_out = vrows * UPR;
+        const bool has_add1 = d.add0 != nullptr && d.add1 != nullptr;
+        f32x8 a0[MAXI], a1[MAXI];
+        if (d.add0) {
+#pragma unroll
+          for (int j = 0; j < MAXI; ++j) {
+            const int v = tid + j * NTHR;
+            if (v < n_out) {
+              a0[j] = Vec8IO<float>::ldg((const float*)d.add0 + g0 + (int64_t)v * 8);
+              if (has_add1) a1[j] = Vec8IO<float>::ldg((const float*)d.add1 + g0 + (int64_t)v * 8);
+            }
+          }
+        }
 #pragma unroll
         for (int j = 0; j < MAXI; ++j) {
-          const int v = threadIdx.x + j * NTHR;
-          if (v < n_out) {
-            a0[j] = Vec8IO<float>::ldg((const float*)d.add0 + g0 + (int64_t)v * 8);
-            if (has_add1) a1[j] = Vec8IO<float>::ldg((const float*)d.add1 + g0 + (int64_t)v * 8);
+          const int v = tid + j * NTHR;
+          if (v >= n_out) continue;
+          const int ro = v / UPR, cu = v - ro * UPR;
+          f32x8 o = Vec8IO<float>::lds(ys + (size_t)ro * pitch + (size_t)cu * 32);
+#pragma unroll
+          for (int e = 0; e < 8; ++e) o[e] = o[e] + xk[j][e];
+          if (d.add0) {
+#pragma unroll
+            for (int e = 0; e < 8; ++e) o[e] = (o[e] + a0[j][e] + (has_add1 ? a1[j][e] : 0.f)) * d.out_scale;
           }
-        }
-      }
-#pragma unroll
-      for (int j = 0; j < MAXI; ++j) {
-        const int v = threadIdx.x + j * NTHR;
-        if (v >= n_out) continue;
-        const int ro = v / UPR, cu = v - ro * UPR;
-        f32x8 o = Vec8IO<float>::lds(ys + (size_t)ro * pitch + (size_t)cu * 32);
-#pragma unroll
-        for (int e = 0; e < 8; ++e) o[e] = o[e] + xk[j][e];
-        if (d.add0) {
-#pragma unroll
-          for (int e = 0; e < 8; ++e) o[e] = (o[e] + a0[j][e] + (has_add1 ? a1[j][e] : 0.f)) * d.out_scale;
-        }
-        float* dst = yg + g0 + (int64_t)v * 8;
-        *reinterpret_cast<f32x4*>(dst) = f32x4{o[0], o[1], o[2], o[3]};
-        *reinterpret_cast<f32x4*>(dst + 4) = f32x4{o[4], o[5], o[6], o[7]};
-      }
-    } else {
-      if (d.add0) unit_store_pass<float, C, keep_small ? 2 : 4, true, NTHR>(d.add0, d.add1, d.out_scale, ys, pitch, vrows, xg, yg, g0);
-      else unit_store_pass<float, C, keep_small ? 4 : 8, false, NTHR>(d.add0, d.add1, d.out_scale, ys, pitch, vrows, xg, yg, g0);
-    }
-  }
-  JATTS_STAMP(7);
+          float* dst = yg + g0 + (int64_t)v * 8;
+          *reinterpret_cast<f32x4*>(dst) = f32x4{o[0], o[1], o[2], o[3]};
+          *reinterpret_cast<f32x4*>(dst + 4) = f32x4{o[4], o[5], o[6], o[7]};
+        }
+      } else {
+        if (d.add0) unit_store_pass<float, C, keep_small ? 2 : 4, true, NTHR>(d.add0, d.add1, d.out_scale, ys, pitch, vrows, xg, yg, g0);
+        else unit_store_pass<float, C, keep_small ? 4 : 8, false, NTHR>(d.add0, d.add1, d.out_scale, ys, pitch, vrows, xg, yg, g0);
+      }
+    }
+    JATTS_STAMP(7);
+    if constexpr (!SLIDE) break;
+    t0 += nout;
+    slide = true;
+    if (t0 >= L) {
+      f_seq += L;
+      if (f_seq >= f_end) break;
+      do { ++b; } while (d.rg.cu_rows[b + 1] == d.rg.cu_rows[b]);
+      t0 = 0;
+      slide = false;
+    } else if (f_seq + t0 >= f_end) {
+      break;
+    }
+  }
   if (tracing) trace[(size_t)wg_lin * 16 + 9] = __builtin_amdgcn_s_memrealtime();
 #undef JATTS_STAMP
 }
 
+inline int resunit16_pick(const jatts_resunit_desc& d, int runs, int wgcols, bool slide_auto, bool slide_fits) {
+  const int64_t positions = ragged_is_1d(d.rg) ? (int64_t)d.rg.total_rows * d.rg.len_mul : (int64_t)d.rg.n_seq * d.rg.max_len * d.rg.len_mul;
+  const bool slide = d.variant == 2 || (d.variant == 0 && slide_auto && positions >= 2 * (int64_t)runs * wgcols);
+  return slide && slide_fits ? 2 : 1;
+}
+
 template <typename T, int C, int WGCOLS, int WN, int WT, int OCC = 2, bool KSPLIT = false, bool RREG = false>
-int launch_resunit_emul16(const jatts_resunit_desc& d, hipStream_t s) {
+int launch_resunit_emul16(const jatts_resunit_desc& d, hipStream_t s, int* pick) {
   const int K = d.k_w, p2 = (K - 1) / 2, p1 = p2 * d.dil;
   const int tt_out = WGCOLS - 2 * p2;
   if (tt_out < 8) return jatts_set_error_msg(JATTS_ERR_UNSUPPORTED, "resunit: kernel too wide for tile");
   const size_t pitch = C * 6 + 16, pitch_x = KSPLIT ? (C / 2) * 6 + 16 : pitch;
   const size_t rows_x = WGCOLS + 2 * p1, rows_h = WGCOLS + K - 1;
   if (KSPLIT && 2 * p1 > 64) return jatts_set_error_msg(JATTS_ERR_UNSUPPORTED, "resunit (emulated, channel halves): halo beyond 32 rows a side");
-  size_t lds = rows_x * pitch_x > rows_h * pitch ? rows_x * pitch_x : rows_h * pitch;
-  const unsigned bias_off = (unsigned)lds;
-  lds += 2 * C * sizeof(float);
+  const size_t region = rows_x * pitch_x > rows_h * pitch ? rows_x * pitch_x : rows_h * pitch;
+  const size_t tail = (size_t)(K - 1) * C * 6;
+  const size_t lds = region + 2 * C * sizeof(float);
   if (lds > 160 * 1024) return jatts_set_error_msg(JATTS_ERR_UNSUPPORTED, "resunit: tile exceeds 160 KiB LDS");
-  const int64_t maxL = (int64_t)d.rg.max_len * d.rg.len_mul;
-  dim3 grid((unsigned)((maxL + tt_out - 1) / tt_out), (unsigned)d.rg.n_seq);
-  if (const int64_t n1 = ragged_tiles_1d(d.rg, tt_out)) grid = dim3((unsigned)n1);
-  auto kern = resunit_emul16_kernel<T, C, WGCOLS, WN, WT, OCC, KSPLIT, RREG>;
-  JATTS_RAISE_LDS_LIMIT(kern);
-  hipLaunchKernelGGL(kern, grid, dim3(WN * WT * 64), lds, s, d, jatts_g_trace, jatts_g_trace_cap, bias_off);
+  int dev = 0, cus = 0;
+  hipError_t e = hipGetDevice(&dev);
+  if (e == hipSuccess) e = hipDeviceGetAttribute(&cus, hipDeviceAttributeMultiprocessorCount, dev);
+  if (e != hipSuccess) return jatts_set_error(e, __FILE__, __LINE__);
+  const int runs = cus * OCC;
+  const int form = resunit16_pick(d, runs, WGCOLS, !RREG, lds + tail <= 160 * 1024);
+  if (pick) {
+    *pick = form;
+    return JATTS_OK;
+  }
+  if (form == 2) {
+    auto kern = resunit_emul16_kernel<T, C, WGCOLS, WN, WT, OCC, KSPLIT, RREG, true>;
+    JATTS_RAISE_LDS_LIMIT(kern);
+    hipLaunchKernelGGL(kern, dim3((unsigned)runs), dim3(WN * WT * 64), lds + tail, s, d, jatts_g_trace, jatts_g_trace_cap, (unsigned)(region + tail));
+  } else {
+    const int64_t maxL = (int64_t)d.rg.max_len * d.rg.len_mul;
+    dim3 grid((unsigned)((maxL + tt_out - 1) / tt_out), (unsigned)d.rg.n_seq);
+    if (const int64_t n1 = ragged_tiles_1d(d.rg, tt_out)) grid = dim3((unsigned)n1);
+    auto kern = resunit_emul16_kernel<T, C, WGCOLS, WN, WT, OCC, KSPLIT, RREG>;
+    JATTS_RAISE_LDS_LIMIT(kern);
+    hipLaunchKernelGGL(kern, grid, dim3(WN * WT * 64), lds, s, d, jatts_g_trace, jatts_g_trace_cap, (unsigned)region);
+  }
   JATTS_CHECK_LAUNCH();
   return JATTS_OK;
 }
diff --git a/jatts_amd/hip.py b/jatts_amd/hip.py
--- a/jatts_amd/hip.py
+++ b/jatts_amd/hip.py
@@ -553,10 +553,9 @@
                              f"pack_conv_weight_bf16x3 with c_mult=32), got {w.numel()} x {w.dtype}")
 
 
-def hifigan_resunit(rb, len_mul, x, y, w1, b1, w2, b2, channels, k_w, dil, slope, dtype, add=None, out_scale=1.0, ws=None, w_layout=0):
-    lib = _abi.load()
+def _resunit_desc(rb, len_mul, x, y, w1, b1, w2, b2, channels, k_w, dil, slope, dtype, add, out_scale, ws, w_layout, variant):
     d = _abi.ResUnitDesc()
-    d.w_layout = w_layout
+    d.w_layout, d.variant = w_layout, variant
     d.rg = rb.struct(len_mul)
     d.dtype, d.channels, d.k_w, d.dil, d.slope = dtype, channels, k_w, dil, slope
     rows = rb.total * len_mul
@@ -576,9 +575,23 @@
         d.add0 = add[0].data_ptr()
         d.add1 = add[1].data_ptr() if len(add) > 1 else None
     d.out_scale = out_scale
-    with _Timed("resunit", (channels, k_w, dil, rows, len(add) if add else 0)):
+    return d
+
+
+def hifigan_resunit(rb, len_mul, x, y, w1, b1, w2, b2, channels, k_w, dil, slope, dtype, add=None, out_scale=1.0, ws=None, w_layout=0, variant=0):
+    lib = _abi.load()
+    d = _resunit_desc(rb, len_mul, x, y, w1, b1, w2, b2, channels, k_w, dil, slope, dtype, add, out_scale, ws, w_layout, variant)
+    with _Timed("resunit", (channels, k_w, dil, rb.total * len_mul, len(add) if add else 0)):
         _abi.check(lib.jatts_hifigan_resunit(C.byref(d), _stream()), "jatts_hifigan_resunit")
     return y
+
+
+def resunit_variant(rb, len_mul, x, y, w1, b1, w2, b2, channels, k_w, dil, slope, dtype, add=None, out_scale=1.0, ws=None, w_layout=0, variant=0):
+    lib = _abi.load()
+    d = _resunit_desc(rb, len_mul, x, y, w1, b1, w2, b2, channels, k_w, dil, slope, dtype, add, out_scale, ws, w_layout, variant)
+    rc = lib.jatts_resunit_variant(C.byref(d))
+    _abi.check(min(rc, 0), "jatts_resunit_variant")
+    return rc
 
 
 def hifigan_resblock(rb, len_mul, x, y, units, channels, k_w, slope, dtype, add=None, out_scale=1.0, ws=None):
```
